# IGNF/MAESTRO

Hardware: AMD Instinct MI355X
Metric: MAE-pretrain tiles/sec (higher is better)
Workload: dtype bf16

## Files before the change

### include/maestro_hip.h

```cpp
#ifndef MAESTRO_HIP_H
#define MAESTRO_HIP_H
#include <stddef.h>
#include <stdint.h>
#ifdef __cplusplus
extern "C" {
#endif

const char* mh_last_error(void);
int mh_version(void);

#define MH_GEMM_OUT_F32 1
#define MH_GEMM_BIAS 2
#define MH_GEMM_GELU 4
#define MH_GEMM_RESIDUAL 8
#define MH_GEMM_DGELU 16
#define MH_GEMM_ATOMIC 32
#define MH_GEMM_COLSUM 64
#define MH_GEMM_AUX_DGELU 128
#define MH_GEMM_MULAUX 256
#define MH_GEMM_AUX_U8 1024
#define MH_GEMM_C8_E5M2 512
#define MH_GEMM_FP8_TILE_256 2048
#define MH_GEMM_FP8_TILE_128 4096
#define MH_GEMM_FP8_TILE_128D 8192
int mh_gemm_bf16(int layout, int M, int N, int K, const void* A, int lda, const void* B, int ldb, void* C, int ldc,
                 int flags, const float* bias, const float* res, int ldr, const void* aux_in, void* aux_out,
                 int ldaux, float* colsum, void* stream);

enum { MH_TILE_AUTO = -1, MH_TILE_REG_128 = 0, MH_TILE_DMA_256 = 1, MH_TILE_DMA_256x128 = 2, MH_TILE_DMA_128x256 = 3,
       MH_TILE_DMA_128 = 4, MH_TILE_DMA_128x4 = 5, MH_TILE_DMA_256_LOCKSTEP = 6, MH_TILE_PP_128 = 7,
       MH_TILE_PP_128_DIAG1 = 8, MH_TILE_PP_128_DIAG2 = 9, MH_TILE_PP_128_DIAG3 = 10,
       MH_TILE_PP_128_DIAG4 = 11, MH_TILE_PP_128_DIAG5 = 12,
       MH_TILE_REG_64 = 13, MH_TILE_REG_192 = 14,
       MH_TILE_SK_192 = 15, MH_TILE_SK_256 = 16,
       MH_TILE_SK_DMA_256 = 17  };
int mh_gemm_bf16_tile(int tile, int layout, int M, int N, int K, const void* A, int lda, const void* B, int ldb, void* C,
                      int ldc, int flags, const float* bias, const float* res, int ldr, const void* aux_in, void* aux_out,
                      int ldaux, float* colsum, void* stream);

#define MH_GEMM_FAMILY_DMA 1
#define MH_GEMM_FAMILY_PP 2
#define MH_GEMM_FAMILY_192 4
#define MH_GEMM_FAMILY_ALL 7
int mh_gemm_bf16_resolve_tile(int tile, int families, int layout, int M, int N, int K, int lda, int ldb, int ldc, int ldr,
                              int ldaux, int flags);

long mh_gemm_sk_workspace(int tile, int grid);
int mh_gemm_bf16_sk(int tile, int layout, int M, int N, int K, const void* A, int lda, const void* B, int ldb, void* C, int ldc,
                    int flags, const float* bias, const float* res, int ldr, void* workspace, long workspace_bytes, int grid,
                    void* stream);

typedef struct MhGroupedGemm {
    const void* A; const void* B; void* C;
    int M, N, K, lda, ldb, ldc, reserved, accumulate;
} MhGroupedGemm;
int mh_gemm_grouped_tn(const MhGroupedGemm* table_device, int n_problems, const uint32_t* tile_queues, int queue_len,
                       void* stream);

enum { MH_FP8_E4M3 = 0, MH_FP8_E5M2 = 1 };
int mh_gemm_fp8(int M, int N, int K, const void* A8, int lda, int a_format, const void* B8, int ldb, void* C, int ldc,
                int flags, const float* descale_a, const float* descale_b, const float* bias, const float* res, int ldr,
                const void* aux_in, void* aux_out, int ldaux, float* colsum, void* c8, int ldc8, const float* c8_scale,
                float* c8_amax, void* stream);
#define MH_FP8_AMAX_SUBSLOTS 32
#define MH_FP8_AMAX_STRIDE 64
#define MH_FP8_AMAX_PITCH (MH_FP8_AMAX_SUBSLOTS * MH_FP8_AMAX_STRIDE)
typedef struct MhQuantJob {
    const void* src; void* dst; void* dst_t;
    long n;
    int rows, cols, slot, is_f32, format, reserved;
} MhQuantJob;
int mh_quant_batched(const MhQuantJob* jobs_device, const unsigned long* items_device, int n_items, const float* scale,
                     float* amax, int mode, void* stream);
int mh_fp8_update_scales(float* amax, float* scale, float* descale, int n, float format_max, int margin_log2, void* stream);
int mh_gemm_mx(int M, int N, int K, const void* A8, int lda, const void* sa, int ldsa, const void* B8, int ldb, const void* sb,
               int ldsb, void* C, int ldc, int flags, const float* bias, const float* res, int ldr, const void* aux_in,
               void* aux_out, int ldaux, float* colsum, void* c8, int ldc8, void* c8_scales, int ldc8s, void* stream);
typedef struct MhQuantMxJob {
    const void* src; void* dst; void* scales;
    int rows, cols, ld_src, ld_dst, ld_s, reserved;
} MhQuantMxJob;
int mh_quant_mx_batched(const MhQuantMxJob* jobs_host, int n_jobs, const MhQuantMxJob* jobs_device, const unsigned long* items_device,
                        int n_items, void* stream);
typedef struct MhTransposeJob { const void* src; void* dst; int rows, cols; } MhTransposeJob;
int mh_transpose_u8_batched(const MhTransposeJob* jobs_device, const unsigned long* items_device, int n_items, void* stream);

int mh_layernorm_fwd(const float* x, int x_L, int x_off, const float* gamma, const float* beta, void* y, int y_L,
                     int y_off, int y_is_f32, float* mean, float* rstd, int B, int n, int dim, float eps, void* stream);
int mh_layernorm_fwd_fp8(const float* x, int x_L, int x_off, const float* gamma, const float* beta, void* y, int y_L,
                         int y_off, float* mean, float* rstd, int B, int n, int dim, float eps, void* y8,
                         const float* y8_scale, float* y8_amax, void* stream);
int mh_layernorm_fwd_mx(const float* x, int x_L, int x_off, const float* gamma, const float* beta, void* y, int y_L, int y_off,
                        float* mean, float* rstd, int B, int n, int dim, float eps, void* y8, void* y8_scales, int ld_y8s,
                        void* stream);
int mh_layernorm_bwd(const void* dy, int dy_L, int dy_off, int dy_is_f32, const float* x, int x_L, int x_off,
                     const float* gamma, const float* mean, const float* rstd, const float* dres, float* dx,
                     void* dx_bf16, float* dgamma, float* dbeta, float* dcol, float* workspace, int B, int n, int dim,
                     void* stream);
long mh_layernorm_bwd_workspace(int rows, int dim);
int mh_layernorm_bwd_partial(const void* dy, int dy_L, int dy_off, int dy_is_f32, const float* x, int x_L, int x_off,
                             const float* gamma, const float* mean, const float* rstd, const float* dres, float* dx,
                             void* dx_bf16, float* workspace, int B, int n, int dim, void* stream);
#define MH_COLSUM_ROWS 16
typedef struct {
    const float* src;
    float* dst;
    int rows, cols, ld, reserved;
} MhColsumJob;
int mh_colsum_batched(const MhColsumJob* jobs_device, int n_jobs, const uint64_t* blocks_device, int n_blocks, void* stream);
#define MH_ORDERED_ROWS 16
#define MH_ORDERED_ADD 1
typedef struct MhOrderedJob {
    const float* src;
    float* dst;
    int rows, cols, ld, flags;
} MhOrderedJob;
int mh_reduce_ordered(const MhOrderedJob* jobs_host, const MhOrderedJob* jobs_device, int n_jobs, const uint64_t* blocks_device,
                      int n_blocks, void* stream);

int mh_attn_fwd(const void* qkv, void* out, float* lse, int B, int N, int H, int D, float scale, void* stream);
int mh_attn_bwd(const void* qkv, const void* out, const void* dout, const float* lse, float* delta, void* dqkv,
                int B, int N, int H, int D, float scale, void* stream);
int mh_patchify(const float* img, void* cols, float* target, int BD, int Ctot, int S, int P, int Kpad,
                const int* norm_bands, int n_norm_groups, int normalise, int rescale_elev, void* stream);
int mh_patchify_bands(const float* img, void* cols, float* target, int BD, int Csrc, int c0, int Ctot, int S, int P, int Kpad,
                      const int* norm_bands, int n_norm_groups, int normalise, int rescale_elev, void* stream);

int mh_groupnorm_stats(const float* y, float* partial, float* stats, int BD, int L, int E, float eps, void* stream);
int mh_groupnorm_partial_size(int BD, int L, int E);
int mh_embed_finish(const float* y, const float* stats, const float* gamma, const float* beta, const float* pos,
                    const float* date, int date_rows, int date_off, float* xg, int B, int D, int L, int E, int tok_off,
                    int Lgroup, void* stream);
int mh_embed_finish_bwd(const float* dxg, const float* y, const float* stats, const float* gamma, void* dyc,
                        float* dgamma, float* dbeta, float* sums, int B, int D, int L, int E, int tok_off, int Lgroup,
                        void* stream);
int mh_embed_bwd_partial_rows(int BD, int L);
int mh_embed_finish_bwd_det(const float* dxg, const float* y, const float* stats, const float* gamma, void* dyc,
                            float* param_partial, float* blk_sums, float* sums, int B, int D, int L, int E, int tok_off, int Lgroup,
                            void* stream);
int mh_embed_bwd_cs_rows(long rows);
int mh_embed_finish_bwd_ends(const float* dx, const int* inv, int n_vis, const float* y, const float* stats, const float* gamma,
                             void* dyc, float* dgamma, float* dbeta, float* sums, float* cs_partial, int B, int D, int L, int E,
                             int tok_off, int Lgroup, void* stream);
int mh_date_features(const int16_t* dates, const int16_t* ref_date, float* out, int B, int D, int rows, int row_off,
                     float fac, void* stream);
int mh_resize(const float* in, float* out, long planes, int Hin, int Win, int Hout, int Wout, int mode, void* stream);
int mh_dihedral(const void* in, void* out, const uint8_t* flags, int B, long planes, int S, int elem_bytes, void* stream);
#define MH_RAW_U8 0
#define MH_RAW_I16 1
#define MH_RAW_U16 2
#define MH_RAW_F32 3
#define MH_SELECT_MAX_WINDOW 64
int mh_select_dates(const void* raw, int raw_code, const unsigned char* mask, int Cm, int mask_floor, const short* dates,
                    const int* t_start, const int* t_win, int w_max, const double* scores, float* out, short* out_dates,
                    int* out_index, int B, int Tmax, int nd, long n_elem, int n_pix, int log_scale, float norm_fac, void* stream);
int mh_rescale_elev(const float* img, float* out, int BD, int C, int S, void* stream);
int mh_depatchify(const float* patches, float* img, int BD, int C, int S, int P, void* stream);

int mh_mask_select(const float* noise, const uint8_t* struct_mask, int* visible_idx, int* masked_idx, int* inv,
                   uint8_t* mask, int B, int L, int k, void* stream);
int mh_gather_rows(const float* src, const int* idx, float* dst, int B, int src_L, int n_idx, int dim, int dst_L,
                   int dst_off, void* stream);
int mh_gather_rows_cs_rows(long rows);
int mh_gather_rows_bf16_cs(const float* src, const int* idx, void* dst16, float* cs_partial, int B, int src_L, int n_idx, int dim,
                           void* stream);
int mh_scatter_rows(const float* ddst, const int* idx, float* dsrc, int B, int src_L, int n_idx, int dim, int dst_L,
                    int dst_off, void* stream);
int mh_expand_rows(const float* src, const int* inv, float* dst, int B, int L, int n, int dim, void* stream);
int mh_unmask_assemble(const float* y, const int* inv, const float* mask_token, const int* tok_slot, const float* pos,
                       const float* date, const int* date_row, int n_date_rows, float* xdec, int B, int L, int n_vis,
                       int Dd, void* stream);
int mh_unmask_token_grad(const float* dxdec, const uint8_t* mask, const int* tok_slot, float* dmask_token, int B, int L,
                         int Dd, int slot, int t_lo, int t_hi, void* stream);
int mh_unmask_assemble_per_sample(const float* y, const int* inv, const float* mask_token, const int* tok_slot_bl,
                                  const float* pos, const float* date, const int* date_row, int n_date_rows, float* xdec,
                                  int B, int L, int n_vis, int Dd, void* stream);
int mh_unmask_token_grad_per_sample(const float* dxdec, const uint8_t* mask, const int* tok_slot_bl, float* dmask_token, int B,
                                    int L, int Dd, int slot, void* stream);
int mh_unmask_token_grad_partial_rows(long n_rows);
int mh_unmask_token_grad_det(const float* dxdec, const uint8_t* mask, const int* tok_slot, float* partial, int B, int L, int Dd,
                             int slot, int t_lo, int t_hi, void* stream);
int mh_unmask_token_grad_per_sample_det(const float* dxdec, const uint8_t* mask, const int* tok_slot_bl, float* partial, int B,
                                        int L, int Dd, int slot, void* stream);
int mh_count_masked(const uint8_t* mask, int B, int L, int t_lo, int t_hi, int* out, void* stream);
int mh_count_masked_elems(const uint8_t* mask, int B, int L, int t_lo, int t_hi, int* out, int mult, int accumulate, void* stream);

int mh_masked_loss(const float* rec, const float* target, const uint8_t* mask_group, const int* n_masked, float weight,
                   float* acc, void* drec, int B, int Lm, int Lgroup, int tok_off, int PPC, int p, void* stream);
int mh_masked_loss_bands(const float* rec, const float* target, const uint8_t* mask_group, const int* n_elems, float weight,
                         float* acc, void* drec, int B, int Lm, int Lgroup, int tok_off, int PPC, int p, int tgt_C, int tgt_c0,
                         int n_g, void* stream);
int mh_masked_loss_partial_size(int B, int Lm);
int mh_masked_loss_det(const float* rec, const float* target, const uint8_t* mask_group, const int* n_masked, float weight,
                       float* loss_partial, void* drec, int B, int Lm, int Lgroup, int tok_off, int PPC, int p, void* stream);
int mh_masked_loss_bands_det(const float* rec, const float* target, const uint8_t* mask_group, const int* n_elems, float weight,
                             float* loss_partial, void* drec, int B, int Lm, int Lgroup, int tok_off, int PPC, int p, int tgt_C,
                             int tgt_c0, int n_g, void* stream);
int mh_masked_loss_cs_rows(int B, int Lm);
int mh_masked_loss_cs(const float* rec, const float* target, const uint8_t* mask_group, const int* n_masked, float weight,
                      float* acc, void* drec, float* cs_partial, int B, int Lm, int Lgroup, int tok_off, int PPC, int p,
                      void* stream);
int mh_masked_loss_bands_cs(const float* rec, const float* target, const uint8_t* mask_group, const int* n_elems, float weight,
                            float* acc, void* drec, float* cs_partial, int B, int Lm, int Lgroup, int tok_off, int PPC, int p,
                            int tgt_C, int tgt_c0, int n_g, void* stream);

int mh_token_resize(const float* in, long in_rows, int in_off, float* out, long out_rows, int out_off, int B, int D, int h,
                    int H, int E, void* stream);
int mh_token_resize_bwd(const float* dout, long out_rows, int out_off, float* din, long in_rows, int in_off, int B, int D,
                        int h, int H, int E, int accumulate, void* stream);
int mh_attn_reduce_fwd(const void* kv, const float* query, float* out, float* lse, int n_batch, int T, int Lr, int dim,
                       int heads, void* stream);
int mh_attn_reduce_bwd(const void* kv, const float* query, const float* out, const float* lse, const float* dout, void* dkv,
                       float* dq_partial, int n_batch, int T, int Lr, int dim, int heads, void* stream);
long mh_attn_reduce_partial_rows(int n_seq);
int mh_mean_reduce_fwd(const float* x, float* out, int n_batch, int T, int Lr, int dim, void* stream);
int mh_mean_reduce_bwd(const float* dout, float* dx, int n_batch, int T, int Lr, int dim, void* stream);
int mh_head_linear_fwd(const float* x, const float* W, const float* bias, float* out, int B, int C, int E, void* stream);
int mh_head_linear_bwd(const float* x, const float* W, const float* dout, float* dx, float* dW, float* db, int B, int C, int E,
                       void* stream);
int mh_count_valid(const void* target, int target_bytes, long n, long missing_val, int* count, void* stream);
int mh_ce_loss(const float* logits, const void* target, int target_bytes, long missing_val, const int* n_valid, float* acc,
               void* dlogits, int dlogits_is_f32, int B, int g, int P, int C, int ld, void* stream);
int mh_bce_loss(const float* logits, const float* target, float missing_val, float* acc, float* dlogits, int B, int C,
                void* stream);
int mh_confusion_ce(const float* logits, const void* target, int target_bytes, long missing_val, long long* cm, int B, int g,
                    int P, int C, int ld, void* stream);
int mh_confusion_bce(const float* logits, const float* target, float missing_val, float logit_threshold, long long* cm, int B,
                     int C, void* stream);

int mh_colsum(const void* x, int x_is_f32, float* out, int M, int N, int ld, void* stream);
#define MH_COLSUM_PARTIAL_ROWS 256
int mh_colsum_partial_rows(int M);
int mh_colsum_partial(const void* x, int x_is_f32, float* partial, int M, int N, int ld, void* stream);
int mh_zero_spans(float* base, const long* spans_device, int n_spans, long max_len, void* stream);
int mh_scale_dev(float* x, long n, const float* scale, void* stream);
int mh_cast_bf16(const float* src, void* dst, long n, void* stream);
int mh_pack_rows_bf16(const float* w, void* dst, int E, int K, int Kpad, void* stream);
int mh_unpack_rows_add(const float* src, float* dst, int E, int K, int Kpad, void* stream);
int mh_adamw(float* p, const float* g, float* m, float* v, void* p_bf16, long n, float lr, float b1, float b2,
             float eps, float wd, int step, float grad_scale, void* stream);
int mh_adamw_fp8(float* p, const float* g, float* m, float* v, void* p_bf16, void* p_fp8, const short* slot_map,
                 const float* scale, float* amax, long n, float lr, float b1, float b2, float eps, float wd, int step,
                 float grad_scale, void* stream);
int mh_adamw_dev(float* p, const float* g, float* m, float* v, void* p_bf16, long n, float b1, float b2, float eps,
                 float wd, const float* hyper, void* stream);

#ifdef __cplusplus
}
#endif
#endif
```

### maestro_amd/csrc/gemm.hip

```cpp
#include "gemm_reg.hpp"

namespace {

template <bool A_KMAJOR, bool B_KMAJOR, int MT = 4>
__global__ __launch_bounds__(NT, MT == 2 ? 3 : 2) void gemm_kernel(GemmParams p) {
    static_assert(!A_KMAJOR || MT == 4, "the K-major A image is 128 columns wide");
    constexpr int TBM = 32 * MT, NA = MT;
    constexpr int A_BYTES = TBM * 128, B_BYTES = TILE_BYTES;
    __shared__ __attribute__((aligned(16))) unsigned char smem[2 * A_BYTES + 2 * B_BYTES];
    unsigned char* const sb = smem + 2 * A_BYTES;
    const int nwg = p.tiles_m * p.tiles_n;
    const int id = xcd_remap(blockIdx.x, nwg);
    constexpr int GROUP_M = MT == 2 ? 16 : 8;
    int tile_m, tile_n;
    raster_tile<GROUP_M>(p, id, tile_m, tile_n);
    const int m0 = tile_m * TBM, n0 = tile_n * BN;
    const int kbeg = blockIdx.y * p.k_per_split;
    const int kend = min(p.K, kbeg + p.k_per_split);
    const int nk = (kend - kbeg + BK - 1) / BK;

    const int w = threadIdx.x >> 6, l = threadIdx.x & 63;
    const int wm = (w >> 1) * (16 * MT), wn = (w & 1) * 64;

    f32x4 acc[4][MT];
#pragma unroll
    for (int j = 0; j < 4; ++j)
#pragma unroll
        for (int i = 0; i < MT; ++i) acc[j][i] = (f32x4){0.f, 0.f, 0.f, 0.f};

    u32x4 ra[NA], rb[4];
    auto mfma_block = [&](const bf16x8 (&fa)[MT], const bf16x8 (&fb)[4]) {
#pragma unroll
        for (int j = 0; j < 4; ++j)
#pragma unroll
            for (int i = 0; i < MT; ++i)
                acc[j][i] = __builtin_amdgcn_mfma_f32_16x16x32_bf16(fb[j], fa[i], acc[j][i], 0, 0, 0);
    };
    auto compute = [&](const unsigned char* ta, const unsigned char* tb) {
#pragma unroll
        for (int s = 0; s < 2; ++s) {
            bf16x8 fa[MT], fb[4];
#pragma unroll
            for (int i = 0; i < MT; ++i) fa[i] = read_frag<A_KMAJOR>(ta, wm + 16 * i, s);
#pragma unroll
            for (int j = 0; j < 4; ++j) fb[j] = read_frag<B_KMAJOR>(tb, wn + 16 * j, s);
            mfma_block(fa, fb);
        }
    };
    auto compute_half = [&](const unsigned char* ta, const unsigned char* tb, int s) {
        bf16x8 fa[MT], fb[4];
#pragma unroll
        for (int i = 0; i < MT; ++i) fa[i] = read_frag<A_KMAJOR>(ta, wm + 16 * i, s);
#pragma unroll
        for (int j = 0; j < 4; ++j) fb[j] = read_frag<B_KMAJOR>(tb, wn + 16 * j, s);
        __builtin_amdgcn_s_setprio(1);
        mfma_block(fa, fb);
        __builtin_amdgcn_s_setprio(0);
    };
    if (p.fast) {
        const __amdgpu_buffer_rsrc_t ra_src = __builtin_amdgcn_make_buffer_rsrc((void*)p.A, (short)0, (int)p.a_bytes, 0x00020000);
        const __amdgpu_buffer_rsrc_t rb_src = __builtin_amdgcn_make_buffer_rsrc((void*)p.B, (short)0, (int)p.b_bytes, 0x00020000);
        int va[NA], vb[4];
        tile_offsets<A_KMAJOR, NA>(p.lda, m0, va);
        tile_offsets<B_KMAJOR>(p.ldb, n0, vb);
        const int a_step = A_KMAJOR ? BK * p.lda * 2 : BK * 2;
        const int b_step = B_KMAJOR ? BK * p.ldb * 2 : BK * 2;
        int a_off = A_KMAJOR ? kbeg * p.lda * 2 : kbeg * 2;
        int b_off = B_KMAJOR ? kbeg * p.ldb * 2 : kbeg * 2;
        load_tile_fast(ra_src, va, a_off, ra);
        load_tile_fast(rb_src, vb, b_off, rb);
        store_tile<A_KMAJOR, NA>(smem, ra);
        store_tile<B_KMAJOR>(sb, rb);
        if (nk > 1) {
            a_off += a_step; b_off += b_step;
            load_tile_fast(ra_src, va, a_off, ra);
            load_tile_fast(rb_src, vb, b_off, rb);
        }
        __syncthreads();
        constexpr int NM = 4 * MT, NS = NA + 4;
        constexpr int NR = (A_KMAJOR ? 8 : MT) + (B_KMAJOR ? 8 : 4);
        int kt0 = 0;
        for (; kt0 + 2 < nk; ++kt0) {
            const int cur = kt0 & 1;
            const unsigned char* ta = smem + cur * A_BYTES;
            const unsigned char* tb = sb + cur * B_BYTES;
            bf16x8 fa[MT], fb[4];
#pragma unroll
            for (int i = 0; i < MT; ++i) fa[i] = read_frag<A_KMAJOR>(ta, wm + 16 * i, 0);
#pragma unroll
            for (int j = 0; j < 4; ++j) fb[j] = read_frag<B_KMAJOR>(tb, wn + 16 * j, 0);
            mfma_block(fa, fb);
            store_tile<A_KMAJOR, NA>(smem + (cur ^ 1) * A_BYTES, ra);
            store_tile<B_KMAJOR>(sb + (cur ^ 1) * B_BYTES, rb);
            a_off += a_step; b_off += b_step;
            load_tile_fast(ra_src, va, a_off, ra);
            load_tile_fast(rb_src, vb, b_off, rb);
#pragma unroll
            for (int i = 0; i < MT; ++i) fa[i] = read_frag<A_KMAJOR>(ta, wm + 16 * i, 1);
#pragma unroll
            for (int j = 0; j < 4; ++j) fb[j] = read_frag<B_KMAJOR>(tb, wn + 16 * j, 1);
            mfma_block(fa, fb);
            __builtin_amdgcn_sched_group_barrier(0x100, NR, 0);
#pragma unroll
            for (int r = 0; r < NS; ++r) {
                __builtin_amdgcn_sched_group_barrier(0x008, NM / NS, 0);
                __builtin_amdgcn_sched_group_barrier(0x200, 1, 0);
                __builtin_amdgcn_sched_group_barrier(0x020, 1, 0);
            }
            if constexpr (NM % NS != 0) __builtin_amdgcn_sched_group_barrier(0x008, NM - (NM / NS) * NS, 0);
            __builtin_amdgcn_sched_group_barrier(0x100, NR, 0);
            __builtin_amdgcn_sched_group_barrier(0x008, NM, 0);
            __syncthreads();
        }
        for (int kt = kt0; kt < nk; ++kt) {
            const int cur = kt & 1;
            const unsigned char* ta = smem + cur * A_BYTES;
            const unsigned char* tb = sb + cur * B_BYTES;
            compute_half(ta, tb, 0);
            if (kt + 1 < nk) {
                store_tile<A_KMAJOR, NA>(smem + (cur ^ 1) * A_BYTES, ra);
                store_tile<B_KMAJOR>(sb + (cur ^ 1) * B_BYTES, rb);
                if (kt + 2 < nk) {
                    a_off += a_step; b_off += b_step;
                    load_tile_fast(ra_src, va, a_off, ra);
                    load_tile_fast(rb_src, vb, b_off, rb);
                }
            }
            compute_half(ta, tb, 1);
            __syncthreads();
        }
    } else {
        unsigned char* ta = smem;
        unsigned char* tb = sb;
        load_tile<A_KMAJOR, NA>(p.A, p.lda, m0, p.M, kbeg, kend, ra);
        load_tile<B_KMAJOR>(p.B, p.ldb, n0, p.N, kbeg, kend, rb);
        store_tile<A_KMAJOR, NA>(ta, ra);
        store_tile<B_KMAJOR>(tb, rb);
        __syncthreads();
        for (int kt = 0; kt < nk; ++kt) {
            const bool more = kt + 1 < nk;
            if (more) {
                load_tile<A_KMAJOR, NA>(p.A, p.lda, m0, p.M, kbeg + (kt + 1) * BK, kend, ra);
                load_tile<B_KMAJOR>(p.B, p.ldb, n0, p.N, kbeg + (kt + 1) * BK, kend, rb);
            }
            compute(ta, tb);
            __syncthreads();
            if (more) {
                store_tile<A_KMAJOR, NA>(ta, ra);
                store_tile<B_KMAJOR>(tb, rb);
            }
            __syncthreads();
        }
    }

    float* st = reinterpret_cast<float*>(smem) + w * (32 * 68);
    if (p.flags & MH_GEMM_ATOMIC) gemm_epilogue_atomic<MT>(p, acc, st, m0 + wm, n0 + wn);
    else gemm_epilogue_store<MT>(p, acc, st, m0 + wm, n0 + wn);
}

}

static int gemm_reg_launch(int tile, int layout, GemmParams& p, hipStream_t s) {
    const int K = p.K;
    const int mt = tile == MH_TILE_REG_64 ? 2 : tile == MH_TILE_REG_192 ? 6 : 4;
    const int tbm = 32 * mt;
    p.tiles_m = ceil_div(p.M, tbm); p.tiles_n = ceil_div(p.N, BN);
    int splits = 1;
    if (p.flags & MH_GEMM_ATOMIC) {
        const int tiles = p.tiles_m * p.tiles_n;
        const int ksteps = ceil_div(K, BK);
        splits = max(1, min(min(512 / max(tiles, 1), ksteps / 4), 32));
    }
    const int ksteps_per = ceil_div(ceil_div(K, BK), splits);
    p.k_per_split = ksteps_per * BK;
    splits = ceil_div(K, p.k_per_split);
    const bool a_kmajor = layout == 2, b_kmajor = layout != 0;
    const long k_rows = (long)ceil_div(K, BK) * BK;
    const bool tail_ok = (a_kmajor && b_kmajor) || K % BK == 0;
    p.fast = tail_ok && gemm_in_reach((a_kmajor ? k_rows : (long)p.tiles_m * tbm) * p.lda * 2, 4096) &&
             gemm_in_reach((b_kmajor ? k_rows : (long)p.tiles_n * BN) * p.ldb * 2, 4096);
    gemm_set_extents(p, layout);
    dim3 grid(p.tiles_m * p.tiles_n, splits), block(NT);
    switch (layout * 8 + mt) {
        case 0 * 8 + 4: hipLaunchKernelGGL((gemm_kernel<false, false, 4>), grid, block, 0, s, p); break;
        case 0 * 8 + 2: hipLaunchKernelGGL((gemm_kernel<false, false, 2>), grid, block, 0, s, p); break;
        case 0 * 8 + 6: hipLaunchKernelGGL((gemm_kernel<false, false, 6>), grid, block, 0, s, p); break;
        case 1 * 8 + 4: hipLaunchKernelGGL((gemm_kernel<false, true, 4>), grid, block, 0, s, p); break;
        case 1 * 8 + 2: hipLaunchKernelGGL((gemm_kernel<false, true, 2>), grid, block, 0, s, p); break;
        case 1 * 8 + 6: hipLaunchKernelGGL((gemm_kernel<false, true, 6>), grid, block, 0, s, p); break;
        default: hipLaunchKernelGGL((gemm_kernel<true, true, 4>), grid, block, 0, s, p); break;
    }
    MH_LAUNCH_CHECK();
    return 0;
}

static int gemm_check_args(bool buffers, int tile, int layout, const GemmParams& p) {
    const int M = p.M, N = p.N, K = p.K, lda = p.lda, ldb = p.ldb, ldc = p.ldc, ldr = p.ldr, ldaux = p.ldaux, flags = p.flags;
    auto given = [&](const void* q) { return !buffers || q; };
    MH_CHECK_ARG(tile >= MH_TILE_AUTO && tile <= MH_TILE_REG_192, "mh_gemm_bf16: tile %d", tile);
    MH_CHECK_ARG(layout >= 0 && layout <= 2, "mh_gemm_bf16: layout %d", layout);
    MH_CHECK_ARG(!(flags & ~0x7ff), "mh_gemm_bf16: unknown flag bits 0x%x", flags & ~0x7ff);
    MH_CHECK_ARG(M > 0 && N > 0 && K > 0, "mh_gemm_bf16: empty problem %d %d %d", M, N, K);
    MH_CHECK_ARG(given(p.A) && given(p.B) && given(p.C), "mh_gemm_bf16: null operand");
    MH_CHECK_ARG(lda % 8 == 0 && ldb % 8 == 0, "mh_gemm_bf16: lda/ldb must be multiples of 8 (%d, %d)", lda, ldb);
    MH_CHECK_ARG(N % 4 == 0 && ldc % 4 == 0, "mh_gemm_bf16: N and ldc must be multiples of 4 (%d, %d)", N, ldc);
    MH_CHECK_ARG((flags & MH_GEMM_OUT_F32) || (N % 8 == 0 && ldc % 8 == 0), "mh_gemm_bf16: bf16 output needs N, ldc %% 8 == 0");
    MH_CHECK_ARG((flags & MH_GEMM_OUT_F32) || !(flags & MH_GEMM_RESIDUAL), "mh_gemm_bf16: residual epilogue needs f32 output");
    MH_CHECK_ARG(!(flags & MH_GEMM_OUT_F32) || !(flags & (MH_GEMM_GELU | MH_GEMM_DGELU | MH_GEMM_MULAUX)), "mh_gemm_bf16: GELU / aux epilogues need bf16 output");
    MH_CHECK_ARG(((uintptr_t)p.A | (uintptr_t)p.B | (uintptr_t)p.C) % 16 == 0, "mh_gemm_bf16: bases must be 16-B aligned");
    if (layout == 2) {
        MH_CHECK_ARG(M % 8 == 0 && N % 8 == 0, "mh_gemm_bf16: TN needs M, N multiples of 8 (%d, %d)", M, N);
    } else {
        MH_CHECK_ARG(K % 8 == 0, "mh_gemm_bf16: K must be a multiple of 8 (%d)", K);
        if (layout == 1) MH_CHECK_ARG(N % 8 == 0, "mh_gemm_bf16: NN needs N multiple of 8 (%d)", N);
    }
    MH_CHECK_ARG(!(flags & MH_GEMM_BIAS) || given(p.bias), "mh_gemm_bf16: bias flag without pointer");
    MH_CHECK_ARG(!(flags & MH_GEMM_RESIDUAL) || (given(p.res) && ldr % 4 == 0), "mh_gemm_bf16: residual needs pointer, ldr%%4==0");
    MH_CHECK_ARG(!(flags & (MH_GEMM_DGELU | MH_GEMM_MULAUX)) || (given(p.aux_in) && ldaux % 8 == 0), "mh_gemm_bf16: dgelu / mulaux need aux_in, ldaux %% 8 == 0");
    MH_CHECK_ARG(!(flags & MH_GEMM_AUX_DGELU) || ((flags & MH_GEMM_GELU) && given(p.aux_out)), "mh_gemm_bf16: aux_dgelu needs the GELU epilogue and aux_out");
    MH_CHECK_ARG(!((flags & MH_GEMM_DGELU) && (flags & MH_GEMM_MULAUX)), "mh_gemm_bf16: dgelu and mulaux exclude each other");
    MH_CHECK_ARG(!(flags & MH_GEMM_AUX_U8) || ((flags & (MH_GEMM_AUX_DGELU | MH_GEMM_MULAUX)) && !(flags & MH_GEMM_DGELU)),
                 "mh_gemm_bf16: MH_GEMM_AUX_U8 applies to the saved GELU derivative only (AUX_DGELU / MULAUX)");
    MH_CHECK_ARG(!(flags & MH_GEMM_GELU) || !p.aux_out || ldaux % 8 == 0, "mh_gemm_bf16: ldaux %% 8");
    MH_CHECK_ARG(!(flags & MH_GEMM_ATOMIC) || (flags & MH_GEMM_OUT_F32), "mh_gemm_bf16: atomic needs f32 output");
    MH_CHECK_ARG(!(flags & MH_GEMM_COLSUM) || (given(p.colsum) && !(flags & MH_GEMM_OUT_F32)), "mh_gemm_bf16: colsum needs a pointer and bf16 output");
    MH_CHECK_ARG(!(flags & MH_GEMM_ATOMIC) || !(flags & ~(MH_GEMM_ATOMIC | MH_GEMM_OUT_F32)),
                 "mh_gemm_bf16: atomic accumulate excludes other epilogues");
    return 0;
}

static bool prefer_dma(int layout, int M, int N, int K, int flags) {
    if (layout == 2 || (flags & MH_GEMM_ATOMIC) || K % 32 != 0 || K < 256) return false;
    const long tiles = (long)ceil_div(M, 256) * ceil_div(N, 256);
    if (tiles < 256) return false;
    const long waves = (tiles + 255) / 256;
    return 10 * tiles >= 9 * 256 * waves;
}

static int gemm_resolve(int tile, int families, int layout, const GemmParams& p) {
    const int M = p.M, N = p.N, K = p.K, flags = p.flags;
    if (tile >= MH_TILE_PP_128 && tile <= MH_TILE_PP_128_DIAG5) return gemm_pp_serves(tile, layout, p) ? tile : -2;
    if (tile > MH_TILE_REG_128 && tile < MH_TILE_PP_128) return gemm_dma_serves(tile, layout, p) ? tile : -2;
    if (tile != MH_TILE_AUTO)
        return layout != 2 && !(flags & MH_GEMM_COLSUM) ? tile : MH_TILE_REG_128;
    const bool dma = (families & MH_GEMM_FAMILY_DMA) && prefer_dma(layout, M, N, K, flags);
    const long t128 = (long)ceil_div(M, 128) * ceil_div(N, 128);
    if ((families & MH_GEMM_FAMILY_192) && !dma && layout != 2 && !(flags & (MH_GEMM_COLSUM | MH_GEMM_ATOMIC)) && K >= 1536 &&
        K % BK == 0 && t128 > 512 && t128 <= 576 && (long)ceil_div(M, 192) * ceil_div(N, 128) <= 512)
        return MH_TILE_REG_192;
    if ((families & MH_GEMM_FAMILY_PP) && !(flags & MH_GEMM_MULAUX) && layout == 0 && t128 >= 256 &&
        ((flags & MH_GEMM_GELU) ? t128 <= 2304 : (!dma || (K < 1024 && t128 <= 8192))) && gemm_pp_serves(MH_TILE_PP_128, layout, p))
        return MH_TILE_PP_128;
    if (dma && gemm_dma_serves(MH_TILE_DMA_256, layout, p)) return MH_TILE_DMA_256;
    return MH_TILE_REG_128;
}

extern "C" int mh_gemm_bf16_resolve_tile(int tile, int families, int layout, int M, int N, int K, int lda, int ldb, int ldc,
                                         int ldr, int ldaux, int flags) {
    GemmParams p;
    gemm_fill(p, M, N, K, nullptr, lda, nullptr, ldb, nullptr, ldc, flags, nullptr, nullptr, ldr, nullptr, nullptr, ldaux, nullptr);
    MH_CHECK_ARG(!(families & ~MH_GEMM_FAMILY_ALL), "mh_gemm_bf16_resolve_tile: unknown family bits 0x%x", families & ~MH_GEMM_FAMILY_ALL);
    if (const int rc = gemm_check_args(false, tile, layout, p)) return rc;
    return gemm_resolve(tile, families, layout, p);
}

extern "C" int mh_gemm_bf16_tile(int tile, int layout, int M, int N, int K, const void* A, int lda, const void* B, int ldb,
                                 void* C, int ldc, int flags, const float* bias, const float* res, int ldr,
                                 const void* aux_in, void* aux_out, int ldaux, float* colsum, void* stream) {
    GemmParams p;
    gemm_fill(p, M, N, K, A, lda, B, ldb, C, ldc, flags, bias, res, ldr, aux_in, aux_out, ldaux, colsum);
    if (const int rc = gemm_check_args(true, tile, layout, p)) return rc;
    const int run = gemm_resolve(tile, MH_GEMM_FAMILY_ALL, layout, p);
    if (run == -2) return -2;
    if (run >= MH_TILE_PP_128 && run <= MH_TILE_PP_128_DIAG5) return gemm_pp_launch(run, layout, p, (hipStream_t)stream);
    if (run > MH_TILE_REG_128 && run < MH_TILE_PP_128) return gemm_dma_launch(run, layout, p, (hipStream_t)stream);
    return gemm_reg_launch(run, layout, p, (hipStream_t)stream);
}

extern "C" int mh_gemm_bf16(int layout, int M, int N, int K, const void* A, int lda, const void* B, int ldb, void* C,
                            int ldc, int flags, const float* bias, const float* res, int ldr, const void* aux_in,
                            void* aux_out, int ldaux, float* colsum, void* stream) {
    return mh_gemm_bf16_tile(MH_TILE_AUTO, layout, M, N, K, A, lda, B, ldb, C, ldc, flags, bias, res, ldr, aux_in, aux_out,
                             ldaux, colsum, stream);
}
```

### maestro_amd/csrc/gemm_dma.hip

```cpp
#include "gemm_ring.hpp"

#ifndef MH_DMA_PRIO
#define MH_DMA_PRIO 0
#endif
#if MH_DMA_PRIO == 0
#define MH_PRIO_UP() __builtin_amdgcn_s_setprio(1)
#define MH_PRIO_DOWN() __builtin_amdgcn_s_setprio(0)
#else
#define MH_PRIO_UP() ((void)0)
#define MH_PRIO_DOWN() ((void)0)
#endif

namespace {

template <class T, bool A_KMAJOR, bool B_KMAJOR, int CALLER, bool STAGGER>
__device__ __forceinline__ void gemm_dma_tile(const GemmParams& p, int tile_m, int tile_n, int kbeg, int kend,
                                              unsigned char* smem) {
    constexpr int S = T::S, PA = T::PA, PB = T::PB, NW = T::NW;
    static_assert(T::LDS_BYTES >= NW * 32 * 68 * 4, "the ring doubles as epilogue staging");
    const int m0 = tile_m * T::BM, n0 = tile_n * T::BN;
    const int nk = (kend - kbeg + BK - 1) / BK;

    const int w = __builtin_amdgcn_readfirstlane(threadIdx.x >> 6), l = threadIdx.x & 63;
    constexpr int MT = T::MT;
    const int wm = (w / T::WN) * (16 * MT), wn = (w % T::WN) * 64;

    const __amdgpu_buffer_rsrc_t ra_src = __builtin_amdgcn_make_buffer_rsrc((void*)p.A, (short)0, (int)p.a_bytes, 0x00020000);
    const __amdgpu_buffer_rsrc_t rb_src = __builtin_amdgcn_make_buffer_rsrc((void*)p.B, (short)0, (int)p.b_bytes, 0x00020000);
    int va[PA], vb[PB];
    piece_offsets<A_KMAJOR, T::BM, NW, PA>(p.lda, m0, w, l, va);
    piece_offsets<B_KMAJOR, T::BN, NW, PB>(p.ldb, n0, w, l, vb);
    const int a_step = A_KMAJOR ? BK * p.lda * 2 : BK * 2;
    const int b_step = B_KMAJOR ? BK * p.ldb * 2 : BK * 2;
    const int a_off0 = A_KMAJOR ? kbeg * p.lda * 2 : kbeg * 2;
    const int b_off0 = B_KMAJOR ? kbeg * p.ldb * 2 : kbeg * 2;

    auto issue = [&](int t) {
        unsigned char* slot = smem + (t % S) * T::STAGE_BYTES;
#pragma unroll
        for (int h = 0; h < PA; ++h)
            __builtin_amdgcn_raw_ptr_buffer_load_lds(ra_src, (lds_void*)(slot + (w + NW * h) * 1024), 16, va[h],
                                                     a_off0 + t * a_step, 0, 0);
#pragma unroll
        for (int h = 0; h < PB; ++h)
            __builtin_amdgcn_raw_ptr_buffer_load_lds(rb_src, (lds_void*)(slot + T::A_BYTES + (w + NW * h) * 1024), 16, vb[h],
                                                     b_off0 + t * b_step, 0, 0);
    };

    f32x4 acc[4][MT];
#pragma unroll
    for (int j = 0; j < 4; ++j)
#pragma unroll
        for (int i = 0; i < MT; ++i) acc[j][i] = (f32x4){0.f, 0.f, 0.f, 0.f};

    for (int t = 0; t < S - 1 && t < nk; ++t) issue(t);

    auto wait_step = [&](int step) {
        const int younger = min(S - 2, nk - 1 - step);
        if (younger >= 2) wait_vmcnt<2 * (PA + PB)>();
        else if (younger == 1) wait_vmcnt<PA + PB>();
        else wait_vmcnt<0>();
    };
    bf16x8 fa[MT], fb[4];
    auto load_step = [&](int t) {
        const unsigned char* ta = smem + (t % S) * T::STAGE_BYTES;
        const unsigned char* tb = ta + T::A_BYTES;
#pragma unroll
        for (int j = 0; j < 4; ++j) fb[j] = read_frag<B_KMAJOR, T::BN>(tb, wn + 16 * j);
#pragma unroll
        for (int i = 0; i < MT; ++i) fa[i] = read_frag<A_KMAJOR, T::BM>(ta, wm + 16 * i);
        __builtin_amdgcn_sched_barrier(0);
        if (t + S - 1 < nk) issue(t + S - 1);
        __builtin_amdgcn_sched_barrier(0);
    };
    auto math_step = [&]() {
#pragma unroll
        for (int i = 0; i < MT; ++i)
#pragma unroll
            for (int j = 0; j < 4; ++j)
                acc[j][i] = __builtin_amdgcn_mfma_f32_16x16x32_bf16(fb[j], fa[i], acc[j][i], 0, 0, 0);
    };

    if constexpr (NW == 8 && STAGGER) {
        wait_step(0);
        __builtin_amdgcn_s_barrier();
#if MH_DMA_PRIO == 1
        if (w >= 4) __builtin_amdgcn_s_setprio(1);
#endif
        if (w < 4) {
            for (int t = 0; t < nk; ++t) {
                load_step(t);
                __builtin_amdgcn_s_barrier();
                __builtin_amdgcn_sched_barrier(0);
                MH_PRIO_UP(); math_step(); MH_PRIO_DOWN();
                if (t + 1 < nk) wait_step(t + 1);
                __builtin_amdgcn_s_barrier();
                __builtin_amdgcn_sched_barrier(0);
            }
        } else {
            __builtin_amdgcn_s_barrier();
            __builtin_amdgcn_sched_barrier(0);
            for (int t = 0; t < nk; ++t) {
                load_step(t);
                if (t + 1 < nk) wait_step(t + 1);
                __builtin_amdgcn_s_barrier();
                __builtin_amdgcn_sched_barrier(0);
                MH_PRIO_UP(); math_step(); MH_PRIO_DOWN();
                if (t + 1 < nk) {
                    __builtin_amdgcn_s_barrier();
                    __builtin_amdgcn_sched_barrier(0);
                }
            }
        }
    } else {
        for (int t = 0; t < nk; ++t) {
            wait_step(t);
            __builtin_amdgcn_s_barrier();
            load_step(t);
            math_step();
        }
        __builtin_amdgcn_s_barrier();
    }

    float* st = reinterpret_cast<float*>(smem) + w * (32 * 68);
    if (p.flags & MH_GEMM_ATOMIC) gemm_epilogue_atomic<MT>(p, acc, st, m0 + wm, n0 + wn);
    else gemm_epilogue_store<MT>(p, acc, st, m0 + wm, n0 + wn);
}

template <class T, bool A_KMAJOR, bool B_KMAJOR, bool STAGGER>
__global__ __launch_bounds__(T::NT, T::MIN_WG) void gemm_dma_kernel(GemmParams p) {
    __shared__ __attribute__((aligned(16))) unsigned char smem[T::LDS_BYTES];
    const int nwg = p.tiles_m * p.tiles_n;
    const int id = xcd_remap(blockIdx.x, nwg);
    int tile_m, tile_n;
    raster_tile<4>(p, id, tile_m, tile_n);
    const int kbeg = blockIdx.y * p.k_per_split;
    gemm_dma_tile<T, A_KMAJOR, B_KMAJOR, 0, STAGGER>(p, tile_m, tile_n, kbeg, min(p.K, kbeg + p.k_per_split), smem);
}

typedef Tile<2, 4, 4> T256;
typedef Tile<2, 2, 3> T256x128;
typedef Tile<1, 4, 3> T128x256;
typedef Tile<1, 2, 4> T128;
typedef Tile<2, 2, 4, 4> T128q;

template <class T, bool STAGGER>
__global__ __launch_bounds__(T::NT) void gemm_dma_grouped_tn_kernel(const MhGroupedGemm* __restrict__ table, int n_problems,
                                                                    const uint32_t* __restrict__ queues, int queue_len) {
    __shared__ __attribute__((aligned(16))) unsigned char smem[T::LDS_BYTES];
    const uint32_t e = queues[(size_t)(blockIdx.x & 7) * queue_len + (blockIdx.x >> 3)];
    if (e == 0xFFFFFFFFu || (int)(e >> 16) >= n_problems) return;
    const MhGroupedGemm g = table[e >> 16];
    GemmParams p;
    p.A = (const bf16_t*)g.A; p.B = (const bf16_t*)g.B; p.C = g.C;
    p.bias = nullptr; p.res = nullptr; p.aux_in = nullptr; p.aux_out = nullptr; p.colsum = nullptr;
    p.M = g.M; p.N = g.N; p.K = g.K; p.lda = g.lda; p.ldb = g.ldb; p.ldc = g.ldc; p.ldr = 0; p.ldaux = 0;
    p.flags = MH_GEMM_OUT_F32 | (g.accumulate ? MH_GEMM_ATOMIC : 0);
    p.tiles_m = (g.M + T::BM - 1) / T::BM; p.tiles_n = (g.N + T::BN - 1) / T::BN; p.k_per_split = g.K; p.fast = 1;
    p.a_bytes = (unsigned)(((long)(g.K - 1) * g.lda + g.M) * 2);
    p.b_bytes = (unsigned)(((long)(g.K - 1) * g.ldb + g.N) * 2);
    const int tile_m = (e >> 8) & 0xff, tile_n = e & 0xff;
    if (tile_m >= p.tiles_m || tile_n >= p.tiles_n) return;
    gemm_dma_tile<T, true, true, 1, STAGGER>(p, tile_m, tile_n, 0, g.K, smem);
}

template <class T>
void launch_dma(int layout, GemmParams& p, hipStream_t s, bool stagger = true) {
    const int K = p.K;
    p.tiles_m = ceil_div(p.M, T::BM); p.tiles_n = ceil_div(p.N, T::BN);
    int splits = 1;
    if (p.flags & MH_GEMM_ATOMIC) {
        const int tiles = p.tiles_m * p.tiles_n, ksteps = ceil_div(K, BK);
        const int slots = 256 * (T::LDS_BYTES > 80 * 1024 ? 1 : 2);
        splits = max(1, min(min(slots / max(tiles, 1), ksteps / 8), 32));
    }
    const int ksteps_per = ceil_div(ceil_div(K, BK), splits);
    p.k_per_split = ksteps_per * BK;
    splits = ceil_div(K, p.k_per_split);
    dim3 grid(p.tiles_m * p.tiles_n, splits), block(T::NT);
    if (T::NW == 8 && stagger) {
        switch (layout) {
            case 0: hipLaunchKernelGGL((gemm_dma_kernel<T, false, false, T::NW == 8>), grid, block, 0, s, p); break;
            case 1: hipLaunchKernelGGL((gemm_dma_kernel<T, false, true, T::NW == 8>), grid, block, 0, s, p); break;
            default: hipLaunchKernelGGL((gemm_dma_kernel<T, true, true, T::NW == 8>), grid, block, 0, s, p); break;
        }
        return;
    }
    switch (layout) {
        case 0: hipLaunchKernelGGL((gemm_dma_kernel<T, false, false, false>), grid, block, 0, s, p); break;
        case 1: hipLaunchKernelGGL((gemm_dma_kernel<T, false, true, false>), grid, block, 0, s, p); break;
        default: hipLaunchKernelGGL((gemm_dma_kernel<T, true, true, false>), grid, block, 0, s, p); break;
    }
}

}

extern "C" int mh_gemm_grouped_tn(const MhGroupedGemm* table_device, int n_problems, const uint32_t* tile_queues,
                                  int queue_len, void* stream) {
    MH_CHECK_ARG(table_device && tile_queues && n_problems > 0 && n_problems < 65536 && queue_len > 0,
                 "mh_gemm_grouped_tn: bad arguments");
    hipLaunchKernelGGL((gemm_dma_grouped_tn_kernel<T256, true>), dim3(8 * queue_len), dim3(T256::NT), 0, (hipStream_t)stream,
                       table_device, n_problems, tile_queues, queue_len);
    MH_LAUNCH_CHECK();
    return 0;
}

bool gemm_dma_serves(int tile, int layout, const GemmParams& p) {
    int bm, bn;
    switch (tile) {
        case MH_TILE_DMA_256: case MH_TILE_DMA_256_LOCKSTEP: bm = T256::BM; bn = T256::BN; break;
        case MH_TILE_DMA_256x128: bm = T256x128::BM; bn = T256x128::BN; break;
        case MH_TILE_DMA_128x256: bm = T128x256::BM; bn = T128x256::BN; break;
        case MH_TILE_DMA_128: case MH_TILE_DMA_128x4: bm = T128::BM; bn = T128::BN; break;
        default: return false;
    }
    const bool a_kmajor = layout == 2, b_kmajor = layout != 0;
    if ((!a_kmajor || !b_kmajor) && p.K % BK != 0) return false;
    const long k_rows = (long)ceil_div(p.K, BK) * BK;
    return gemm_in_reach((a_kmajor ? k_rows : (long)ceil_div(p.M, bm) * bm) * p.lda * 2) &&
           gemm_in_reach((b_kmajor ? k_rows : (long)ceil_div(p.N, bn) * bn) * p.ldb * 2);
}

int gemm_dma_launch(int tile, int layout, GemmParams& p, hipStream_t s) {
    p.fast = 1;
    gemm_set_extents(p, layout);
    switch (tile) {
        case MH_TILE_DMA_256: launch_dma<T256>(layout, p, s); break;
        case MH_TILE_DMA_256x128: launch_dma<T256x128>(layout, p, s); break;
        case MH_TILE_DMA_128x256: launch_dma<T128x256>(layout, p, s); break;
        case MH_TILE_DMA_128: launch_dma<T128>(layout, p, s); break;
        case MH_TILE_DMA_128x4: launch_dma<T128q>(layout, p, s); break;
        default: launch_dma<T256>(layout, p, s, false); break;
    }
    MH_LAUNCH_CHECK();
    return 0;
}
```

### maestro_amd/csrc/gemm_pp.hip

```cpp
#include "gemm_reg.hpp"
#include <type_traits>

#ifndef MH_PP_PRIO
#define MH_PP_PRIO 1
#endif

namespace {

enum { EPI_BF16 = 0, EPI_GELU = 1, EPI_MULAUX = 2, EPI_F32 = 3 };
constexpr int EPI_STEPS = 8;

__device__ __forceinline__ void swap16(uint32_t& a, uint32_t& b) {
    const u32x2 r = __builtin_amdgcn_permlane16_swap(a, b, false, false);
    a = r[0]; b = r[1];
}

template <bool B_KMAJOR, int EPI, int DIAG = 0>
__global__ __launch_bounds__(NT, 2) void gemm_pp_kernel(GemmParams p) {
    __shared__ __attribute__((aligned(16))) unsigned char smem[4 * TILE_BYTES];
    const int T = p.tiles_m * p.tiles_n, G = gridDim.x;
    const int x = blockIdx.x & 7, slot = blockIdx.x >> 3, per_x = G >> 3;
    const int q = T >> 3, r8 = T & 7;
    const int run0 = x < r8 ? x * (q + 1) : r8 * (q + 1) + (x - r8) * q;
    const int cnt = q + (x < r8 ? 1 : 0);
    if (slot >= cnt) return;
    const int n_my = (cnt - slot + per_x - 1) / per_x;
    const int nk = p.K / BK;
    auto coords = [&](int t, int& m0, int& n0) {
        int tm, tn;
        raster_tile<8>(p, run0 + slot + t * per_x, tm, tn);
        m0 = tm * BM;
        n0 = tn * BN;
    };

    const int tid = threadIdx.x, w = tid >> 6, l = tid & 63, g = l >> 4, lm = l & 15;
    const int wm = (w >> 1) * 64, wn = (w & 1) * 64;

    const __amdgpu_buffer_rsrc_t ra_src = __builtin_amdgcn_make_buffer_rsrc((void*)p.A, (short)0, (int)p.a_bytes, 0x00020000);
    const __amdgpu_buffer_rsrc_t rb_src = __builtin_amdgcn_make_buffer_rsrc((void*)p.B, (short)0, (int)p.b_bytes, 0x00020000);
    const int a_v0 = ((tid >> 3) * p.lda + (tid & 7) * 8) * 2;
    const int b_v0 = B_KMAJOR ? ((tid >> 4) * p.ldb + (tid & 15) * 8) * 2 : ((tid >> 3) * p.ldb + (tid & 7) * 8) * 2;
    const int a_i = 32 * p.lda * 2, b_i = (B_KMAJOR ? 16 : 32) * p.ldb * 2;
    const int a_step = BK * 2, b_step = B_KMAJOR ? BK * p.ldb * 2 : BK * 2;
    int ld_kt = 0, ld_m0, ld_n0, nx_m0, nx_n0;
    coords(0, ld_m0, ld_n0);
    coords(min(1, n_my - 1), nx_m0, nx_n0);
    u32x4 ra[4], rb[4];
    auto issue_loads = [&]() {
        const int a_t = ld_m0 * p.lda * 2, b_t = B_KMAJOR ? ld_n0 * 2 : ld_n0 * p.ldb * 2;
        const int a_k = ld_kt * a_step, b_k = ld_kt * b_step;
#pragma unroll
        for (int i = 0; i < 4; ++i) ra[i] = __builtin_amdgcn_raw_buffer_load_b128(ra_src, a_v0 + (a_t + i * a_i), a_k, 0);
#pragma unroll
        for (int i = 0; i < 4; ++i) rb[i] = __builtin_amdgcn_raw_buffer_load_b128(rb_src, b_v0 + (b_t + i * b_i), b_k, 0);
    };
    auto advance = [&]() {
        const bool wrap = ++ld_kt == nk;
        ld_kt = wrap ? 0 : ld_kt;
        ld_m0 = wrap ? nx_m0 : ld_m0;
        ld_n0 = wrap ? nx_n0 : ld_n0;
    };

    f32x4 acc[4][4], prev[4][4];
    int sidx = 0;

    const __amdgpu_buffer_rsrc_t rc_dst = __builtin_amdgcn_make_buffer_rsrc(
        p.C, (short)0, (int)(((long)(p.M - 1) * p.ldc + p.N) * (EPI == EPI_F32 ? 4 : 2)), 0x00020000);
    const __amdgpu_buffer_rsrc_t raux = __builtin_amdgcn_make_buffer_rsrc(
        EPI == EPI_GELU ? (void*)p.aux_out : EPI == EPI_MULAUX ? (void*)p.aux_in : (void*)p.res, (short)0,
        (int)(EPI == EPI_F32 ? ((long)(p.M - 1) * p.ldr + p.N) * 4 : EPI == EPI_BF16 ? 0 : (long)(p.M - 1) * p.ldaux + p.N), 0x00020000);
    const __amdgpu_buffer_rsrc_t rbias = __builtin_amdgcn_make_buffer_rsrc((void*)p.bias, (short)0, p.bias ? p.N * 4 : 0, 0x00020000);
    const __amdgpu_buffer_rsrc_t rcs = __builtin_amdgcn_make_buffer_rsrc(
        (void*)p.colsum, (short)0, EPI == EPI_MULAUX ? (int)((long)((p.M + 63) / 64) * p.N * 4) : 0, 0x00020000);
    const int w_s = __builtin_amdgcn_readfirstlane(w);
    int e_c = 0, e_aux = 0, e_bias = 0, e_cs = 0;
    f32x4 bias_x = {0, 0, 0, 0}, bias_y = {0, 0, 0, 0};
    f32x4 cs_x = {0, 0, 0, 0}, cs_y = {0, 0, 0, 0};
    u32x4 ld_x = {0, 0, 0, 0}, ld_y = {0, 0, 0, 0};
    auto epi_setup = [&](int m0, int n0) {
        int lane = __builtin_amdgcn_mbcnt_hi(~0u, __builtin_amdgcn_mbcnt_lo(~0u, 0u));
        asm volatile("" : "+v"(lane));
        const int g = lane >> 4, lm = lane & 15;
        const int wm = (w_s >> 1) * 64, wn = (w_s & 1) * 64;
        const int col_nat = wn + 4 * g;
        const int col_swp = wn + 4 * g + 12 * (g & 1);
        const int row = m0 + wm + lm;
        if constexpr (EPI == EPI_F32) {
            e_c = (row * p.ldc + n0 + col_nat) * 4;
            e_aux = (row * p.ldr + n0 + col_nat) * 4;
        } else {
            e_c = (row * p.ldc + n0 + col_swp) * 2;
            e_aux = row * p.ldaux + n0 + (EPI == EPI_GELU ? col_swp : col_nat);
        }
        e_bias = (n0 + col_nat) * 4;
        e_cs = (((m0 + wm) >> 6) * p.N + n0 + col_nat) * 4;
    };
    auto epi_loads = [&](auto cc) {
        constexpr int c = decltype(cc)::value, jp = c >> 2, i = c & 3;
        if constexpr (DIAG == 1) return;
        if constexpr (EPI == EPI_GELU || EPI == EPI_F32) {
            if constexpr (i == 0) {
                bias_x = __builtin_bit_cast(f32x4, __builtin_amdgcn_raw_buffer_load_b128(rbias, e_bias + 128 * jp, 0, 0));
                bias_y = __builtin_bit_cast(f32x4, __builtin_amdgcn_raw_buffer_load_b128(rbias, e_bias + 128 * jp + 64, 0, 0));
            }
        }
        if constexpr (EPI == EPI_F32) {
            const int o = e_aux + (16 * i * p.ldr + 32 * jp) * 4;
            ld_x = __builtin_amdgcn_raw_buffer_load_b128(raux, o, 0, 0);
            ld_y = __builtin_amdgcn_raw_buffer_load_b128(raux, o + 64, 0, 0);
        }
        if constexpr (EPI == EPI_MULAUX) {
            const int o = e_aux + 16 * i * p.ldaux + 32 * jp;
            ld_x[0] = __builtin_amdgcn_raw_buffer_load_b32(raux, o, 0, 0);
            ld_y[0] = __builtin_amdgcn_raw_buffer_load_b32(raux, o + 16, 0, 0);
        }
    };
    auto epi_math = [&](auto cc, const f32x4 (&src)[4][4]) {
        constexpr int c = decltype(cc)::value, jp = c >> 2, i = c & 3;
        f32x4 vx = src[2 * jp][i], vy = src[2 * jp + 1][i];
        if constexpr (DIAG == 1) {
            asm volatile("" ::"v"(vx), "v"(vy));
            return;
        }
        if constexpr (EPI == EPI_F32) {
            const int o = e_c + (16 * i * p.ldc + 32 * jp) * 4;
            vx = vx + (bias_x + __builtin_bit_cast(f32x4, ld_x));
            vy = vy + (bias_y + __builtin_bit_cast(f32x4, ld_y));
            __builtin_amdgcn_raw_buffer_store_b128(__builtin_bit_cast(u32x4, vx), rc_dst, o, 0, 0);
            __builtin_amdgcn_raw_buffer_store_b128(__builtin_bit_cast(u32x4, vy), rc_dst, o + 64, 0, 0);
            return;
        } else {
            if constexpr (EPI == EPI_GELU) {
                vx += bias_x; vy += bias_y;
                f32x4 cx, dx, cy, dy;
                if constexpr (DIAG == 3) { cx = vx; dx = vx; cy = vy; dy = vy; }
                else { gelu_cdf_pdf4(vx, cx, dx); gelu_cdf_pdf4(vy, cy, dy); }
                const f32x4 gx = vx * dx + cx, gy = vy * dy + cy;
                uint32_t bx = 0, by = 0;
#pragma unroll
                for (int e = 0; e < 4; ++e) {
                    bx = __builtin_amdgcn_cvt_pk_u8_f32(__builtin_fmaf(gx[e], 200.f, 26.f), e, bx);
                    by = __builtin_amdgcn_cvt_pk_u8_f32(__builtin_fmaf(gy[e], 200.f, 26.f), e, by);
                }
                swap16(bx, by);
                if constexpr (DIAG == 2) asm volatile("" ::"v"(bx), "v"(by));
                else __builtin_amdgcn_raw_buffer_store_b64((u32x2){bx, by}, raux, e_aux + 16 * i * p.ldaux + 32 * jp, 0, 0);
                vx *= cx; vy *= cy;
            }
            if constexpr (EPI == EPI_MULAUX) {
                vx *= unpack_dgelu_u8x4(ld_x[0]);
                vy *= unpack_dgelu_u8x4(ld_y[0]);
                if constexpr (i == 0) { cs_x = vx; cs_y = vy; } else { cs_x += vx; cs_y += vy; }
                if constexpr (i == 3) {
#pragma unroll
                    for (int o = 1; o < 16; o <<= 1) {
#pragma unroll
                        for (int e = 0; e < 4; ++e) {
                            cs_x[e] += __shfl_xor(cs_x[e], o, 64);
                            cs_y[e] += __shfl_xor(cs_y[e], o, 64);
                        }
                    }
                    __builtin_amdgcn_raw_buffer_store_b128(__builtin_bit_cast(u32x4, cs_x), rcs, e_cs + 128 * jp, 0, 0);
                    __builtin_amdgcn_raw_buffer_store_b128(__builtin_bit_cast(u32x4, cs_y), rcs, e_cs + 128 * jp + 64, 0, 0);
                }
            }
            uint32_t x0 = pack_bf2(vx[0], vx[1]), x1 = pack_bf2(vx[2], vx[3]);
            uint32_t y0 = pack_bf2(vy[0], vy[1]), y1 = pack_bf2(vy[2], vy[3]);
            swap16(x0, y0);
            swap16(x1, y1);
            if constexpr (DIAG == 2) asm volatile("" ::"v"(x0), "v"(x1), "v"(y0), "v"(y1));
            else __builtin_amdgcn_raw_buffer_store_b128((u32x4){x0, x1, y0, y1}, rc_dst, e_c + (16 * i * p.ldc + 32 * jp) * 2, 0, 0);
        }
    };

    auto kstep = [&](auto first_c, auto chunk_c) {
        constexpr bool FIRST = decltype(first_c)::value;
        constexpr int CHUNK = decltype(chunk_c)::value;
        const int cur = sidx & 1;
        const unsigned char* ta = smem + cur * TILE_BYTES;
        const unsigned char* tb = smem + (2 + cur) * TILE_BYTES;
        bf16x8 fa[4], fb[4];
#if MH_PP_PRIO == 2
        __builtin_amdgcn_s_setprio(1);
#endif
#pragma unroll
        for (int i = 0; i < 4; ++i) fa[i] = read_frag<false>(ta, wm + 16 * i, 0);
#pragma unroll
        for (int j = 0; j < 4; ++j) fb[j] = read_frag<B_KMAJOR>(tb, wn + 16 * j, 0);
        if constexpr (CHUNK >= 0) epi_loads(chunk_c);
#if MH_PP_PRIO == 1 || MH_PP_PRIO == 3
        __builtin_amdgcn_s_setprio(MH_PP_PRIO);
#endif
#pragma unroll
        for (int j = 0; j < 4; ++j)
#pragma unroll
            for (int i = 0; i < 4; ++i)
                acc[j][i] = __builtin_amdgcn_mfma_f32_16x16x32_bf16(fb[j], fa[i], FIRST ? (f32x4){0.f, 0.f, 0.f, 0.f} : acc[j][i], 0, 0, 0);
        store_tile<false>(smem + (cur ^ 1) * TILE_BYTES, ra);
        store_tile<B_KMAJOR>(smem + (2 + (cur ^ 1)) * TILE_BYTES, rb);
        issue_loads();
#pragma unroll
        for (int i = 0; i < 4; ++i) fa[i] = read_frag<false>(ta, wm + 16 * i, 1);
#pragma unroll
        for (int j = 0; j < 4; ++j) fb[j] = read_frag<B_KMAJOR>(tb, wn + 16 * j, 1);
#pragma unroll
        for (int j = 0; j < 4; ++j)
#pragma unroll
            for (int i = 0; i < 4; ++i)
                acc[j][i] = __builtin_amdgcn_mfma_f32_16x16x32_bf16(fb[j], fa[i], acc[j][i], 0, 0, 0);
        if constexpr (CHUNK >= 0) epi_math(chunk_c, prev);
        constexpr int NV0 = CHUNK < 0 ? 0 : EPI == EPI_GELU ? 14 : EPI == EPI_MULAUX ? 6 : EPI == EPI_F32 ? 2 : 2;
        constexpr int NV = DIAG == 4 ? NV0 : DIAG == 5 ? (NV0 * 4 + 6) / 7 : 0;
        constexpr int NR = DIAG == 5 ? NV0 * 2 : 0;
        __builtin_amdgcn_sched_group_barrier(0x100, B_KMAJOR ? 12 : 8, 0);
        if constexpr (NR > 0) __builtin_amdgcn_sched_group_barrier(0x402, NR, 0);
        constexpr int NL = CHUNK < 0 ? 0 : (EPI == EPI_F32 || EPI == EPI_MULAUX ? 2 : 0) + ((EPI == EPI_F32 || EPI == EPI_GELU) && (CHUNK & 3) == 0 ? 2 : 0);
        if constexpr (NL > 0) __builtin_amdgcn_sched_group_barrier(0x020, NL, 0);
#pragma unroll
        for (int r = 0; r < 8; ++r) {
            __builtin_amdgcn_sched_group_barrier(0x008, 2, 0);
            __builtin_amdgcn_sched_group_barrier(0x200, 1, 0);
            __builtin_amdgcn_sched_group_barrier(0x020, 1, 0);
            if constexpr (NV > 0) __builtin_amdgcn_sched_group_barrier(0x402, NV, 0);
        }
        __builtin_amdgcn_sched_group_barrier(0x100, B_KMAJOR ? 12 : 8, 0);
        if constexpr (NR > 0) __builtin_amdgcn_sched_group_barrier(0x402, NR, 0);
#pragma unroll
        for (int r = 0; r < 8; ++r) {
            __builtin_amdgcn_sched_group_barrier(0x008, 2, 0);
            if constexpr (NV > 0) __builtin_amdgcn_sched_group_barrier(0x402, NV, 0);
        }
        ++sidx;
#if MH_PP_PRIO
        __builtin_amdgcn_s_setprio(0);
#endif
        __syncthreads();
        advance();
    };
    using std::integral_constant;
    constexpr integral_constant<bool, true> kFirst{};
    constexpr integral_constant<bool, false> kNext{};
    constexpr integral_constant<int, -1> kNone{};

    issue_loads(); advance();
    store_tile<false>(smem, ra);
    store_tile<B_KMAJOR>(smem + 2 * TILE_BYTES, rb);
    issue_loads();
    __syncthreads();
    advance();

    int cm0, cn0;
    coords(0, cm0, cn0);
    kstep(kFirst, kNone);
    for (int kt = 1; kt < nk; ++kt) kstep(kNext, kNone);
    for (int t = 1; t < n_my; ++t) {
#pragma unroll
        for (int j = 0; j < 4; ++j)
#pragma unroll
            for (int i = 0; i < 4; ++i) prev[j][i] = acc[j][i];
        epi_setup(cm0, cn0);
        coords(t, cm0, cn0);
        coords(min(t + 1, n_my - 1), nx_m0, nx_n0);
        kstep(kFirst, integral_constant<int, 0>{});
        kstep(kNext, integral_constant<int, 1>{});
        kstep(kNext, integral_constant<int, 2>{});
        kstep(kNext, integral_constant<int, 3>{});
        kstep(kNext, integral_constant<int, 4>{});
        kstep(kNext, integral_constant<int, 5>{});
        kstep(kNext, integral_constant<int, 6>{});
        kstep(kNext, integral_constant<int, 7>{});
        for (int kt = EPI_STEPS; kt < nk; ++kt) kstep(kNext, kNone);
    }
    epi_setup(cm0, cn0);
    if constexpr (DIAG == 0 && (EPI == EPI_F32 || EPI == EPI_MULAUX)) {
        u32x4 tx[8], ty[8];
        f32x4 tbx[2] = {{0, 0, 0, 0}, {0, 0, 0, 0}}, tby[2] = {{0, 0, 0, 0}, {0, 0, 0, 0}};
        auto fetch = [&](auto cc) {
            constexpr int c = decltype(cc)::value;
            epi_loads(cc);
            tx[c] = ld_x; ty[c] = ld_y;
            if constexpr ((c & 3) == 0) { tbx[c >> 2] = bias_x; tby[c >> 2] = bias_y; }
        };
        auto finish = [&](auto cc) {
            constexpr int c = decltype(cc)::value;
            ld_x = tx[c]; ld_y = ty[c]; bias_x = tbx[c >> 2]; bias_y = tby[c >> 2];
            epi_math(cc, acc);
        };
        fetch(integral_constant<int, 0>{}); fetch(integral_constant<int, 1>{}); fetch(integral_constant<int, 2>{});
        fetch(integral_constant<int, 3>{}); fetch(integral_constant<int, 4>{}); fetch(integral_constant<int, 5>{});
        fetch(integral_constant<int, 6>{}); fetch(integral_constant<int, 7>{});
        finish(integral_constant<int, 0>{}); finish(integral_constant<int, 1>{}); finish(integral_constant<int, 2>{});
        finish(integral_constant<int, 3>{}); finish(integral_constant<int, 4>{}); finish(integral_constant<int, 5>{});
        finish(integral_constant<int, 6>{}); finish(integral_constant<int, 7>{});
    } else {
        auto tail = [&](auto cc) { epi_loads(cc); epi_math(cc, acc); };
        tail(integral_constant<int, 0>{}); tail(integral_constant<int, 1>{}); tail(integral_constant<int, 2>{});
        tail(integral_constant<int, 3>{}); tail(integral_constant<int, 4>{}); tail(integral_constant<int, 5>{});
        tail(integral_constant<int, 6>{}); tail(integral_constant<int, 7>{});
    }
}

template <bool B_KMAJOR>
void launch_pp(int epi, int grid, const GemmParams& p, hipStream_t s, int diag = 0) {
    dim3 g(grid), b(NT);
#ifdef MH_DIAG_TILES
    if constexpr (!B_KMAJOR) {
        if (diag == 1 && epi == EPI_GELU) { hipLaunchKernelGGL((gemm_pp_kernel<false, EPI_GELU, 1>), g, b, 0, s, p); return; }
        if (diag == 2 && epi == EPI_GELU) { hipLaunchKernelGGL((gemm_pp_kernel<false, EPI_GELU, 2>), g, b, 0, s, p); return; }
        if (diag == 3 && epi == EPI_GELU) { hipLaunchKernelGGL((gemm_pp_kernel<false, EPI_GELU, 3>), g, b, 0, s, p); return; }
        if (diag == 4 && epi == EPI_GELU) { hipLaunchKernelGGL((gemm_pp_kernel<false, EPI_GELU, 4>), g, b, 0, s, p); return; }
        if (diag == 5 && epi == EPI_GELU) { hipLaunchKernelGGL((gemm_pp_kernel<false, EPI_GELU, 5>), g, b, 0, s, p); return; }
        if (diag == 1 && epi == EPI_BF16) { hipLaunchKernelGGL((gemm_pp_kernel<false, EPI_BF16, 1>), g, b, 0, s, p); return; }
    }
#else
    (void)diag;
#endif
    switch (epi) {
        case EPI_BF16: hipLaunchKernelGGL((gemm_pp_kernel<B_KMAJOR, EPI_BF16>), g, b, 0, s, p); break;
        case EPI_GELU: hipLaunchKernelGGL((gemm_pp_kernel<B_KMAJOR, EPI_GELU>), g, b, 0, s, p); break;
        case EPI_MULAUX: hipLaunchKernelGGL((gemm_pp_kernel<B_KMAJOR, EPI_MULAUX>), g, b, 0, s, p); break;
        default: hipLaunchKernelGGL((gemm_pp_kernel<B_KMAJOR, EPI_F32>), g, b, 0, s, p); break;
    }
}

}

static int pp_epilogue(int flags) {
    if (flags == 0) return EPI_BF16;
    if (flags == (MH_GEMM_BIAS | MH_GEMM_GELU | MH_GEMM_AUX_DGELU | MH_GEMM_AUX_U8)) return EPI_GELU;
    if (flags == (MH_GEMM_MULAUX | MH_GEMM_AUX_U8 | MH_GEMM_COLSUM)) return EPI_MULAUX;
    if (flags == (MH_GEMM_OUT_F32 | MH_GEMM_BIAS | MH_GEMM_RESIDUAL)) return EPI_F32;
    return -1;
}

bool gemm_pp_serves(int tile, int layout, const GemmParams& p) {
    const int epi = pp_epilogue(p.flags), diag = tile - MH_TILE_PP_128;
#ifndef MH_DIAG_TILES
    if (diag != 0) return false;
#else
    if (diag != 0 && (layout != 0 || !(epi == EPI_GELU || (epi == EPI_BF16 && diag == 1)))) return false;
#endif
    if (epi < 0 || layout == 2 || p.K % BK != 0 || p.K < EPI_STEPS * BK || p.N % BN != 0) return false;
    const long rows = (long)ceil_div(p.M, BM) * BM;
    return gemm_in_reach(rows * p.lda * 2) && gemm_in_reach((long)(layout == 1 ? p.K : p.N) * p.ldb * 2) &&
           gemm_in_reach(rows * p.ldc * (epi == EPI_F32 ? 4 : 2)) && gemm_in_reach(epi == EPI_F32 ? rows * p.ldr * 4 : rows * p.ldaux);
}

int gemm_pp_launch(int tile, int layout, GemmParams& p, hipStream_t stream) {
    p.tiles_m = ceil_div(p.M, BM); p.tiles_n = p.N / BN; p.k_per_split = p.K; p.fast = 1;
    gemm_set_extents(p, layout);
    const int tiles = p.tiles_m * p.tiles_n;
#ifndef MH_PP_TILES_PER_WG
#define MH_PP_TILES_PER_WG 0
#endif
    int grid = tiles >= 512 ? 512 : (tiles + 7) / 8 * 8;
    if (MH_PP_TILES_PER_WG > 0) grid = max(grid, ((tiles + MH_PP_TILES_PER_WG - 1) / MH_PP_TILES_PER_WG + 7) / 8 * 8);
    if (layout == 1) launch_pp<true>(pp_epilogue(p.flags), grid, p, stream);
    else launch_pp<false>(pp_epilogue(p.flags), grid, p, stream, tile - MH_TILE_PP_128);
    MH_LAUNCH_CHECK();
    return 0;
}
```

### maestro_amd/engine.py

```python

from __future__ import annotations

import contextlib
import gc
import os
import weakref
import time

import torch
from torch import nn

from maestro_amd import hip
from maestro_amd.fp8 import mx_scale_cols, resolve_scaling
from maestro_amd.layers.utils import draw_struct_masks

F32, BF16, I32, U8 = torch.float32, torch.bfloat16, torch.int32, torch.uint8
_NEVER = object()
_ROCTX = os.environ.get("MAESTRO_ROCTX", "0") == "1"
RING = 4
ALIGN = 64


class ParamStore:

# ... 154 lines not shown
            s, x_in, x_mid, x_out = self.saved[l], self.xs[2 * l], self.xs[2 * l + 1], self.xs[2 * l + 2]
            if self.f8 is not None:
                self._forward_layer_fp8(l, attn, ff, s, x_in, x_mid, x_out)
                continue
            proj = attn.to_out[0]
            hip.layernorm_fwd(x_in, M, 0, attn.norm.weight, attn.norm.bias, s["h1"], M, 0, s["mean1"], s["rstd1"], 1, M, dim)
            hip.gemm(hip.GEMM_NT, M, 3 * inner, dim, s["h1"], dim, ps.h(attn.to_qkv.weight), dim, s["qkv"], 3 * inner)
            hip.attn_fwd(s["qkv"], s["o"], s["lse"], self.Bn, self.N, self.H, self.Dh, attn.scale)
            hip.gemm(hip.GEMM_NT, M, dim, inner, s["o"], inner, ps.h(proj.weight), inner, x_mid, dim,
                     hip.OUT_F32 | hip.BIAS | hip.RESIDUAL, bias=proj.bias, res=x_in, ldr=dim)
            ln2, fc1, fc2 = ff.net[0], ff.net[1], ff.net[4]
            hip.layernorm_fwd(x_mid, M, 0, ln2.weight, ln2.bias, s["h2"], M, 0, s["mean2"], s["rstd2"], 1, M, dim)
            hip.gemm(hip.GEMM_NT, M, mlp, dim, s["h2"], dim, ps.h(fc1.weight), dim, s["act"], mlp,
                     hip.BIAS | hip.GELU | hip.AUX_DGELU | eng.aux_flag, bias=fc1.bias, aux_out=s["hpre"], ldaux=mlp)
            hip.gemm(hip.GEMM_NT, M, dim, mlp, s["act"], mlp, ps.h(fc2.weight), mlp, x_out, dim,
                     hip.OUT_F32 | hip.BIAS | hip.RESIDUAL, bias=fc2.bias, res=x_mid, ldr=dim)

    def _forward_layer_fp8(self, l, attn, ff, s, x_in, x_mid, x_out) -> None:
        eng, M, dim, mlp, inner = self.eng, self.M, self.dim, self.mlp, self.inner
        plan, f = eng.fp8, self.f8[l]
        proj, ln2, fc1, fc2 = attn.to_out[0], ff.net[0], ff.net[1], ff.net[4]
        fc1_flags = hip.BIAS | hip.GELU | hip.AUX_DGELU | eng.aux_flag
        res_flags = hip.OUT_F32 | hip.BIAS | hip.RESIDUAL
        if plan.scaling == "mx":
            ws = plan.w_scales
            ld = lambda t: t.stride(0)
            hip.layernorm_fwd_mx(x_in, M, 0, attn.norm.weight, attn.norm.bias, s["h1"], M, 0, s["mean1"], s["rstd1"], 1, M, dim,
                                 f["h1"], f["mx_h1"], ld(f["mx_h1"]))
            hip.gemm_mx(M, 3 * inner, dim, f["h1"], dim, f["mx_h1"], ld(f["mx_h1"]), f["w_qkv"], dim, ws(f["sw_qkv"]), dim // 32,
                        s["qkv"], 3 * inner)
            hip.attn_fwd(s["qkv"], s["o"], s["lse"], self.Bn, self.N, self.H, self.Dh, attn.scale)
            plan.quantize_mx(s["o"], f["o"], f["mx_o"])
            hip.gemm_mx(M, dim, inner, f["o"], inner, f["mx_o"], ld(f["mx_o"]), f["w_proj"], inner, ws(f["sw_proj"]), inner // 32,
                        x_mid, dim, flags=res_flags, bias=proj.bias, res=x_in, ldr=dim)
            hip.layernorm_fwd_mx(x_mid, M, 0, ln2.weight, ln2.bias, s["h2"], M, 0, s["mean2"], s["rstd2"], 1, M, dim, f["h2"],
                                 f["mx_h2"], ld(f["mx_h2"]))
            hip.gemm_mx(M, mlp, dim, f["h2"], dim, f["mx_h2"], ld(f["mx_h2"]), f["w_fc1"], dim, ws(f["sw_fc1"]), dim // 32,
                        s["act"], mlp, flags=fc1_flags, bias=fc1.bias, aux_out=s["hpre"], ldaux=mlp, c8=f["act"], ldc8=mlp,
                        c8_scales=f["mx_act"], ldc8s=ld(f["mx_act"]))
            hip.gemm_mx(M, dim, mlp, f["act"], mlp, f["mx_act"], ld(f["mx_act"]), f["w_fc2"], mlp, ws(f["sw_fc2"]), mlp // 32,
                        x_out, dim, flags=res_flags, bias=fc2.bias, res=x_mid, ldr=dim)
            return
        hip.layernorm_fwd_fp8(x_in, M, 0, attn.norm.weight, attn.norm.bias, s["h1"], M, 0, s["mean1"], s["rstd1"], 1, M, dim,
                              f["h1"], plan.a_scale(f["s_h1"]), plan.a_amax(f["s_h1"]))
        hip.gemm_fp8(M, 3 * inner, dim, f["h1"], dim, f["w_qkv"], dim, s["qkv"], 3 * inner, plan.a_descale(f["s_h1"]),
                     plan.w_descale(f["sw_qkv"]))
        hip.attn_fwd(s["qkv"], s["o"], s["lse"], self.Bn, self.N, self.H, self.Dh, attn.scale)
        plan.quantize(s["o"], f["o"], f["s_o"])
        hip.gemm_fp8(M, dim, inner, f["o"], inner, f["w_proj"], inner, x_mid, dim, plan.a_descale(f["s_o"]),
                     plan.w_descale(f["sw_proj"]), flags=res_flags, bias=proj.bias, res=x_in, ldr=dim)
        hip.layernorm_fwd_fp8(x_mid, M, 0, ln2.weight, ln2.bias, s["h2"], M, 0, s["mean2"], s["rstd2"], 1, M, dim, f["h2"],
                              plan.a_scale(f["s_h2"]), plan.a_amax(f["s_h2"]))
        hip.gemm_fp8(M, mlp, dim, f["h2"], dim, f["w_fc1"], dim, s["act"], mlp, plan.a_descale(f["s_h2"]),
                     plan.w_descale(f["sw_fc1"]), flags=fc1_flags, bias=fc1.bias, aux_out=s["hpre"],
                     ldaux=mlp, c8=f["act"], ldc8=mlp, c8_scale=plan.a_scale(f["s_act"]), c8_amax=plan.a_amax(f["s_act"]))
        hip.gemm_fp8(M, dim, mlp, f["act"], mlp, f["w_fc2"], mlp, x_out, dim, plan.a_descale(f["s_act"]),
                     plan.w_descale(f["sw_fc2"]), flags=res_flags, bias=fc2.bias, res=x_mid, ldr=dim)

    def reduce_jobs(self, lo: int = 0, hi: int | None = None) -> list:
        ps, dim, mlp, jobs = self.eng.store, self.dim, self.mlp, []
        for l in range(lo, self.depth if hi is None else hi):
            attn, ff = self.t.layers[l]
            s, ln2, fc1, proj = self.saved[l], ff.net[0], ff.net[1], attn.to_out[0]
            jobs.append((s["cs"], ps.g(fc1.bias), self.cs_rows, mlp, mlp))
            for ws, norm, bias in ((s["ws2"], ln2, ps.g(proj.bias)),
                                   (s["ws1"], attn.norm, ps.g(self.t.layers[l - 1][1].net[4].bias) if l > 0 else None)):
                flat = ws.view(-1)
                jobs.append((flat, ps.g(norm.weight), self.ln_rows, dim, 3 * dim))
                jobs.append((flat[dim:], ps.g(norm.bias), self.ln_rows, dim, 3 * dim))
                if bias is not None:
                    jobs.append((flat[2 * dim:], bias, self.ln_rows, dim, 3 * dim))
        return jobs

    def wgrad_problems(self, lo: int = 0, hi: int | None = None) -> list:
        ps, M = self.eng.store, self.M
        dim, mlp, inner = self.dim, self.mlp, self.inner
        out = []
        for l in range(lo, self.depth if hi is None else hi):
            attn, ff = self.t.layers[l]
            s, fc1, fc2, proj = self.saved[l], ff.net[1], ff.net[4], attn.to_out[0]
            out += [(s["gy16"], s["act"], ps.g(fc2.weight), dim, mlp, M, dim, mlp, mlp),
                    (s["dh"], s["h2"], ps.g(fc1.weight), mlp, dim, M, mlp, dim, dim),
                    (s["gmid16"], s["o"], ps.g(proj.weight), dim, inner, M, dim, inner, inner),
                    (s["dqkv"], s["h1"], ps.g(attn.to_qkv.weight), 3 * inner, dim, M, 3 * inner, dim, dim)]
        return out

    def backward(self, dx_out: torch.Tensor, hi: int | None = None, lo: int = 0, defer: bool = False, ready: bool = True):
        eng, ps, M = self.eng, self.eng.store, self.M
        dim, mlp, inner = self.dim, self.mlp, self.inner
        AT = hip.OUT_F32 | hip.ATOMIC
        cur = dx_out
        hi = self.depth if hi is None else hi
        cur16 = self.saved[hi - 1]["gy16"] if hi > 0 else self.dx0_16
        for l in reversed(range(lo, hi)):
            attn, ff = self.t.layers[l]
            s, x_in, x_mid = self.saved[l], self.xs[2 * l], self.xs[2 * l + 1]
            ln2, fc1, fc2 = ff.net[0], ff.net[1], ff.net[4]
            proj = attn.to_out[0]
            cur16, mid16, dh, dqkv = s["gy16"], s["gmid16"], s["dh"], s["dqkv"]
            mid = self.dxa if cur is not self.dxa else self.dxb
            nxt = self.dxa if mid is not self.dxa else self.dxb
            nxt16 = self.saved[l - 1]["gy16"] if l > 0 else self.dx0_16
            f = self.f8[l] if self.f8 is not None and self.f8[l]["dgrad"] else None
            plan = getattr(eng, "fp8", None)
            f8 = f is not None and plan.grad_ready
            if f is not None:
                plan.quantize_grad(cur16, f["gy8"], f["g_gy"])
            if f8:
                hip.gemm_fp8(M, mlp, dim, f["gy8"], dim, f["wt_fc2"], dim, dh, mlp, plan.g_descale(f["g_gy"]),
                             plan.w_descale(f["sw_fc2"]), flags=hip.MULAUX | hip.COLSUM | hip.C8_E5M2 | eng.aux_flag, a_format=hip.FP8_E5M2,
                             aux_in=s["hpre"], ldaux=mlp, colsum=s["cs"] if defer else self.cs_ws, c8=f["dh8"], ldc8=mlp,
                             c8_scale=plan.g_scale(f["g_dh"]), c8_amax=plan.g_amax(f["g_dh"]))
            else:
                hip.gemm(hip.GEMM_NN, M, mlp, dim, cur16, dim, ps.h(fc2.weight), mlp, dh, mlp, hip.MULAUX | hip.COLSUM | eng.aux_flag,
                         aux_in=s["hpre"], ldaux=mlp, colsum=s["cs"] if defer else self.cs_ws)
                if f is not None:
                    plan.quantize_grad(dh, f["dh8"], f["g_dh"])
            if not defer:
                hip.colsum(self.cs_ws, ps.g(fc1.bias), self.cs_rows, mlp, mlp)
                hip.gemm(hip.GEMM_TN, dim, mlp, M, cur16, dim, s["act"], mlp, ps.g(fc2.weight), mlp, AT)
                hip.gemm(hip.GEMM_TN, mlp, dim, M, dh, mlp, s["h2"], dim, ps.g(fc1.weight), dim, AT)
            if f8:
                hip.gemm_fp8(M, dim, mlp, f["dh8"], mlp, f["wt_fc1"], mlp, self.dh2, dim, plan.g_descale(f["g_dh"]),
                             plan.w_descale(f["sw_fc1"]), a_format=hip.FP8_E5M2)
            else:
                hip.gemm(hip.GEMM_NN, M, dim, mlp, dh, mlp, ps.h(fc1.weight), dim, self.dh2, dim)
            if defer:
                hip.layernorm_bwd_partial(self.dh2, M, 0, x_mid, M, 0, ln2.weight, s["mean2"], s["rstd2"], cur, mid, mid16, s["ws2"],
                                          1, M, dim)
            else:
                hip.layernorm_bwd(self.dh2, M, 0, x_mid, M, 0, ln2.weight, s["mean2"], s["rstd2"], cur, mid, mid16,
                                  ps.g(ln2.weight), ps.g(ln2.bias), ps.g(proj.bias), self.ln_ws, 1, M, dim)
            if f is not None:
                plan.quantize_grad(mid16, f["mid8"], f["g_mid"])
            if f8:
                hip.gemm_fp8(M, inner, dim, f["mid8"], dim, f["wt_proj"], dim, self.do, inner, plan.g_descale(f["g_mid"]),
                             plan.w_descale(f["sw_proj"]), a_format=hip.FP8_E5M2)
            else:
                hip.gemm(hip.GEMM_NN, M, inner, dim, mid16, dim, ps.h(proj.weight), inner, self.do, inner)
            if not defer:
                hip.gemm(hip.GEMM_TN, dim, inner, M, mid16, dim, s["o"], inner, ps.g(proj.weight), inner, AT)
            hip.attn_bwd(s["qkv"], s["o"], self.do, s["lse"], self.delta, dqkv, self.Bn, self.N, self.H, self.Dh, attn.scale)
            if not defer:
                hip.gemm(hip.GEMM_TN, 3 * inner, dim, M, dqkv, 3 * inner, s["h1"], dim, ps.g(attn.to_qkv.weight), dim, AT)
            if f is not None:
                plan.quantize_grad(dqkv, f["dqkv8"], f["g_dqkv"])
            if f8:
                hip.gemm_fp8(M, dim, 3 * inner, f["dqkv8"], 3 * inner, f["wt_qkv"], 3 * inner, self.dh2, dim,
                             plan.g_descale(f["g_dqkv"]), plan.w_descale(f["sw_qkv"]), a_format=hip.FP8_E5M2)
            else:
                hip.gemm(hip.GEMM_NN, M, dim, 3 * inner, dqkv, 3 * inner, ps.h(attn.to_qkv.weight), dim, self.dh2, dim)
            prev_fc2_bias = ps.g(self.t.layers[l - 1][1].net[4].bias) if l > 0 else None
            if defer:
                hip.layernorm_bwd_partial(self.dh2, M, 0, x_in, M, 0, attn.norm.weight, s["mean1"], s["rstd1"], mid, nxt, nxt16,
                                          s["ws1"], 1, M, dim)
            else:
                hip.layernorm_bwd(self.dh2, M, 0, x_in, M, 0, attn.norm.weight, s["mean1"], s["rstd1"], mid, nxt, nxt16,
                                  ps.g(attn.norm.weight), ps.g(attn.norm.bias), prev_fc2_bias, self.ln_ws, 1, M, dim)
            cur, cur16 = nxt, nxt16
            if ready:
                eng._grads_ready(self.t.layers[l])
        return cur, cur16


class PatchEmbedEnd:

    def __init__(self, eng: "EngineBase", s) -> None:
        self.eng, self.s = eng, s
        m, dev, E = eng.model, eng.device, eng.E
        e = lambda *sh, dt=F32: torch.empty(*sh, dtype=dt, device=dev)
        z = lambda *sh, dt=F32: torch.zeros(*sh, dtype=dt, device=dev)
        T, BD = s.Beff * s.n_tok, s.Beff * s.D
        self.buf = dict(
            cols=e(T, s.Kpad, dt=BF16), yconv=e(T, E), gn_partial=e(hip.groupnorm_partial_size(BD, s.L, E)), gn_stats=e(BD, 2),
            gn_sums=e(BD, 2), pos_enc=m.pos_enc_rows[s.name].to(dev), norm_bands=torch.tensor(s.norm_bands, dtype=I32, device=dev),
            w_conv16=z(E, s.Kpad, dt=BF16), dw_conv=z(E, s.Kpad), dyc=e(T, E, dt=BF16),
            pe=m.patch_embed[s.embed].patchify_bands[s.gi])

    def pack(self) -> None:
        b, s = self.buf, self.s
        hip.pack_rows_bf16(b["pe"].conv.weight, b["w_conv16"], self.eng.E, s.K, s.Kpad)

    def forward(self, batch: dict, gbuf: dict, xg: torch.Tensor, Lgroup: int, target=None, normalise: bool = False) -> None:
        eng, s, b = self.eng, self.s, self.buf
        m, B, E = eng.model, eng.B, eng.E
        BD, T = s.Beff * s.D, s.Beff * s.n_tok
        if s.G == 1 and target is not None:
            hip.patchify(batch[s.src], b["cols"], target, BD, s.C, s.S, s.P, s.Kpad, b["norm_bands"], len(s.norm_bands),
                         normalise, s.rescale_elev)
        else:
            hip.patchify_bands(batch[s.src], b["cols"], None, BD, s.C_src, s.c0, s.C, s.S, s.P, s.Kpad, None, 0, False,
                               s.rescale_elev)
            if target is not None and s.gi == 0:
                k_src = s.C_src * s.P * s.P
                hip.patchify_bands(batch[s.src], None, target, BD, s.C_src, 0, s.C_src, s.S, s.P, (k_src + 7) // 8 * 8,
                                   b["norm_bands"], len(s.norm_bands), normalise, s.rescale_elev)
        dates, ref_date = batch[f"{s.src}_dates"], batch["ref_date"]
        if s.D != s.Dates:
            hip.date_features(dates, ref_date, gbuf["dates"].view(B, s.Dates, 8), B, s.Dates, s.Dates, 0, m.fac_date_enc)
        else:
            hip.date_features(dates, ref_date, gbuf["dates"], B, s.D, gbuf["n_dates"], s.date_off, m.fac_date_enc)
        pe = b["pe"]
        hip.gemm(hip.GEMM_NT, T, E, s.Kpad, b["cols"], s.Kpad, b["w_conv16"], s.Kpad, b["yconv"], E, hip.OUT_F32 | hip.BIAS,
                 bias=pe.conv.bias)
        hip.groupnorm_stats(b["yconv"], b["gn_partial"], b["gn_stats"], BD, s.L, E)
        hip.embed_finish(b["yconv"], b["gn_stats"], pe.norm.weight, pe.norm.bias, b["pos_enc"], gbuf["dates"], gbuf["n_dates"],
                         s.date_off, xg, s.Beff, s.D, s.L, E, s.tok_off, Lgroup)

    def backward(self, dxg: torch.Tensor, Lgroup: int, clear_dw: bool, defer_wgrad: bool = False) -> None:
        eng, s, b = self.eng, self.s, self.buf
        ps, E, pe, T = eng.store, eng.E, b["pe"], s.Beff * s.n_tok
        if getattr(eng, "deterministic", False):
            return self._backward_det(dxg, Lgroup)
        hip.embed_finish_bwd(dxg, b["yconv"], b["gn_stats"], pe.norm.weight, b["dyc"], ps.g(pe.norm.weight), ps.g(pe.norm.bias),
                             b["gn_sums"], s.Beff, s.D, s.L, E, s.tok_off, Lgroup)
        if not defer_wgrad:
            self._wgrad_in_line(clear_dw)
        hip.colsum(b["dyc"], ps.g(pe.conv.bias), T, E, E)

    def _wgrad_in_line(self, clear_dw: bool) -> None:
        eng, s, b = self.eng, self.s, self.buf
        E, T = eng.E, s.Beff * s.n_tok
        if clear_dw:
            b["dw_conv"].zero_()
        hip.gemm(hip.GEMM_TN, E, s.Kpad, T, b["dyc"], E, b["cols"], s.Kpad, b["dw_conv"], s.Kpad, hip.OUT_F32 | hip.ATOMIC)
        hip.unpack_rows_add(b["dw_conv"], eng.store.g(b["pe"].conv.weight), E, s.K, s.Kpad)

    def wgrad_problem(self) -> tuple:
        b, s, E = self.buf, self.s, self.eng.E
        return (b["dyc"], b["cols"], b["dw_conv"], E, s.Kpad, s.Beff * s.n_tok, E, s.Kpad, s.Kpad)

    def cs_buffer(self) -> torch.Tensor:
        b, s = self.buf, self.s
        if b.get("dyc_cs") is None:
            b["dyc_cs"] = torch.empty(hip.embed_bwd_cs_rows(s.Beff * s.n_tok), self.eng.E, dtype=F32, device=self.eng.device)
        return b["dyc_cs"]

    def backward_ends(self, dx: torch.Tensor, inv, n_vis: int, Lgroup: int, defer_wgrad: bool, clear_dw: bool) -> None:
        eng, s, b = self.eng, self.s, self.buf
        ps, E, pe = eng.store, eng.E, b["pe"]
        hip.embed_finish_bwd_ends(dx, inv, n_vis, b["yconv"], b["gn_stats"], pe.norm.weight, b["dyc"], ps.g(pe.norm.weight),
                                  ps.g(pe.norm.bias), b["gn_sums"], self.cs_buffer(), s.Beff, s.D, s.L, E, s.tok_off, Lgroup)
        if not defer_wgrad:
            self._wgrad_in_line(clear_dw)

    def _backward_det(self, dxg: torch.Tensor, Lgroup: int) -> None:
        eng, s, b = self.eng, self.s, self.buf
        ps, E, pe, T = eng.store, eng.E, b["pe"], s.Beff * s.n_tok

        def make():
            e = lambda *sh: torch.empty(*sh, dtype=F32, device=eng.device)
            rows, S, cr = hip.embed_bwd_partial_rows(s.Beff * s.D, s.L), hip.det_slices(T), hip.colsum_partial_rows(T)
            w = dict(gn=e(rows, 2 * E), blk=e(rows, 2), slabs=e(S, E, s.Kpad), cs=e(cr, E))
            flat = w["gn"].view(-1)
            return w, [(flat, ps.g(pe.norm.weight), rows, E, 2 * E), (flat[E:], ps.g(pe.norm.bias), rows, E, 2 * E),
                       (w["slabs"].view(-1), b["dw_conv"].view(-1), S, E * s.Kpad, E * s.Kpad),
                       (w["cs"].view(-1), ps.g(pe.conv.bias), cr, E, E)]
        w = eng._det_site("bwd", ("embed", s.name), make)
        hip.embed_finish_bwd_det(dxg, b["yconv"], b["gn_stats"], pe.norm.weight, b["dyc"], w["gn"], w["blk"], b["gn_sums"], s.Beff,
                                 s.D, s.L, E, s.tok_off, Lgroup)
        hip.gemm_tn_slabs(E, s.Kpad, T, b["dyc"], E, b["cols"], s.Kpad, w["slabs"])
        hip.colsum_partial(b["dyc"], w["cs"], T, E, E)


_RETIRED_GRAPHS: list = []


def resolve_deterministic(flag: bool | None = None) -> bool:
    if flag is None:
        return os.environ.get("MAESTRO_DETERMINISTIC", "0") == "1"
    return bool(flag)


def training_warm_passes() -> int:
    return 0 if _PROCESS_WARMED else max(0, int(os.environ.get("MAESTRO_WARM_PASSES", "6")))


def _retire_graphs(graphs: dict) -> None:
    if graphs:
        _RETIRED_GRAPHS.append(dict(graphs))
        graphs.clear()


def drain_retired_graphs() -> None:
    if _RETIRED_GRAPHS:
        torch.cuda.synchronize()
        _RETIRED_GRAPHS.clear()


_PROCESS_WARMED = False


class EngineBase:

    def _init_runtime(self, device, n_side_streams: int) -> None:
        self.device = device
        self.grad_hook = None
        self.use_graphs = os.environ.get("MAESTRO_GRAPHS", "1") != "0"
        self.tie_order = os.environ.get("MAESTRO_TIE_ORDER", "stable")
        self.multi_stream = True
        self.group_streams = os.environ.get("MAESTRO_GROUP_STREAMS") != "0"
        self.tune_gemm = os.environ.get("MAESTRO_TUNE", "0") == "1"
        self.instep_tune = (os.environ.get("MAESTRO_INSTEP_TUNE", "0") == "1" and not self.tune_gemm
                            and not any(os.environ.get(k) for k in ("MH_GEMM_TILE", "MH_GEMM_DMA", "MH_GEMM_PP", "MH_DMA_STAGGER")))
        self.tile_report = None
        self.warm_passes = 0
        self.warm_passes_run = 0
        self.aux_flag = hip.AUX_U8 if os.environ.get("MAESTRO_AUX_U8", "1") == "1" else 0
        self._tuned = set()
        gc.collect()
        if os.environ.get("MAESTRO_KEEP_RETIRED_GRAPHS", "0") != "1":
            drain_retired_graphs()
        self._graphs, self._seen, self._ready_spans = {}, {}, []
        weakref.finalize(self, _retire_graphs, self._graphs)
        self._inputs = {}
        prio = int(os.environ.get("MAESTRO_SIDE_PRIORITY", "0"))
        self.side_streams = [torch.cuda.Stream(device=device, priority=prio) for _ in range(max(0, n_side_streams))]
        self._wgrad_stream = torch.cuda.Stream(device=device)
        self._wgrad_tables = {}
        self._dw_conv_clear = False

    def _stable_inputs(self, batch: dict) -> dict:
        out = {}
        for k, t in batch.items():
            if not isinstance(t, torch.Tensor) or not t.is_cuda:
                out[k] = t
                continue
            st = self._inputs.get(k)
            if st is None:
                self._inputs[k] = {"ptr": t.data_ptr(), "buf": None}
                out[k] = t
            elif st["buf"] is None and st["ptr"] == t.data_ptr():
                out[k] = t
            else:
                buf = st["buf"]
                if buf is None or buf.shape != t.shape or buf.dtype != t.dtype:
                    buf = st["buf"] = torch.empty_like(t, memory_format=torch.contiguous_format)
                if buf.data_ptr() != t.data_ptr():
                    buf.copy_(t)
                out[k] = buf
        return out

    def _alloc_embed(self) -> None:
        self.embed = {name: PatchEmbedEnd(self, s) for name, s in self.mods.items()}
        self.mb = {name: end.buf for name, end in self.embed.items()}

    def _pack_conv_weights(self) -> None:
        for end in self.embed.values():
            end.pack()

    def _stage_inputs(self, batch: dict) -> dict:
        sources = [parts[0] for parts in self.model.src_specs.values()]
        for s in sources:
            img = batch[s.src]
            if img.dtype != F32 or not img.is_contiguous() or not img.is_cuda:
                raise ValueError(f"batch[{s.src!r}] must be a contiguous float32 GPU tensor")
            d = batch[f"{s.src}_dates"]
            if d.dtype != torch.int16 or not d.is_contiguous():
                raise ValueError(f"batch['{s.src}_dates'] must be a contiguous int16 tensor [B, D, 3]")
        batch = self._stable_inputs(batch)
        for s in sources:
            img = batch[s.src]
            if tuple(img.shape[-2:]) != (s.S, s.S) or self.model.interpolate != "nearest":
                mode = {"nearest": 0, "bilinear": 1, "bicubic": 2}.get(self.model.interpolate)
                if mode is None:
                    raise ValueError(f"Invalid interpolate mode {self.model.interpolate!r} (nearest, bilinear, bicubic)")
                buf = self.mb[s.name].get("resized")
                if buf is None:
                    buf = self.mb[s.name]["resized"] = torch.empty(self.B, s.Dates, s.C_src, s.S, s.S, dtype=F32, device=self.device)
                hip.resize(img, buf, self.B * s.Dates * s.C_src, img.shape[-2], img.shape[-1], s.S, s.S, mode)
                batch[s.src] = buf
        self._staged = batch
        self._cur_key = tuple(batch[k].data_ptr() for k in sorted(batch) if isinstance(batch[k], torch.Tensor))
        return batch

    def returned_batch(self, batch: dict) -> dict:
        out = dict(batch)
        sources = [parts[0] for parts in self.model.src_specs.values()]
        out.update({s.src: self._staged[s.src] for s in sources})
        for s in sources:
            if s.rescale_elev:
                img = out[s.src]
                res = torch.empty_like(img)
                hip.rescale_elev(img, res, img.shape[0] * img.shape[1], s.C_src, s.S)
                out[s.src] = res
        return out

    def _grads_ready(self, module) -> None:
        ps = list(module.parameters())
        if ps:
            self._ready_spans.append(self.store.span(ps))

    def _run_parallel(self, fns) -> None:
        if len(fns) == 1 or not self.multi_stream or not self.group_streams:
            for fn in fns:
                fn()
            return
        main = torch.cuda.current_stream()
        sides = self.side_streams[: len(fns) - 1]
        for side in sides:
            side.wait_stream(main)
        fns[0]()
        for side, fn in zip(sides, fns[1:]):
            with torch.cuda.stream(side):
                fn()
        for side in sides:
            main.wait_stream(side)

    def _instep_tune(self, one_pass) -> None:
        self.instep_tune = False
        if (getattr(self, "fp8", None) is not None or getattr(self, "_opt", None) is not None or hip.kernel_timer_active()
                or torch.cuda.is_current_stream_capturing()):
            return
        saved = (self.use_graphs, self.multi_stream, self.grad_hook)
        self.use_graphs, self.multi_stream, self.grad_hook = False, False, None
        tuner = hip.InStepTuner()
        hip.set_instep_tuner(tuner)
        try:
            one_pass()
            for cand in tuner.CANDIDATES:
                tuner.begin(cand)
                one_pass()
            tuner.begin(None)
            self.tile_report = tuner.finish()
        finally:
            hip.set_instep_tuner(None)
            self.use_graphs, self.multi_stream, self.grad_hook = saved

    def _warm_up(self, one_pass) -> None:
        global _PROCESS_WARMED
        n, self.warm_passes = self.warm_passes, 0
        self.warm_passes_run = 0
        if (n <= 0 or _PROCESS_WARMED or getattr(self, "fp8", None) is not None or getattr(self, "_opt", None) is not None
                or hip.kernel_timer_active() or torch.cuda.is_current_stream_capturing() or not torch.is_grad_enabled()):
            return
        _PROCESS_WARMED = True
        hook, graphs = self.grad_hook, self.use_graphs
        self.use_graphs = False
        if hook is not None:
            self.grad_hook = lambda lo, hi: None
        try:
            for _ in range(n):
                one_pass()
                self.warm_passes_run += 1
        finally:
            self.grad_hook, self.use_graphs = hook, graphs

    def _first_step_passes(self, one_pass) -> None:
        if self.instep_tune:
            self._instep_tune(one_pass)
        if self.warm_passes > 0:
            self._warm_up(one_pass)

    def _launch_wgrads(self, items, ends=()) -> None:
        items = [(st, lo, hi) for st, lo, hi in items if hi > lo]
        if not items and not ends:
            return
        key = (tuple((st.tag, lo, hi) for st, lo, hi in items), tuple(ends))
        table = self._wgrad_tables.get(key)
        if table is None:
            if torch.cuda.is_current_stream_capturing():
                raise hip.HipExtensionError(f"weight-gradient table {key} first needed inside a hipGraph capture")
            probs = [p for st, lo, hi in items for p in st.wgrad_problems(lo, hi)]
            jobs = [j for st, lo, hi in items for j in st.reduce_jobs(lo, hi)]
            after, ready = [], []
            for tag in ends:
                e_probs, e_jobs, e_after, e_ready = self._ends_table(tag)
                probs, jobs, after, ready = probs + e_probs, jobs + e_jobs, after + e_after, ready + e_ready
            table = self._wgrad_tables[key] = (hip.GroupedTN(probs, self.device) if probs else None,
                                               hip.ColsumBatch(jobs, self.device) if jobs else None, after, ready)
        if table[1] is not None:
            table[1].launch()
        if table[0] is not None:
            table[0].launch()
        for fn in table[2]:
            fn()
        for module in table[3]:
            self._grads_ready(module)

    @contextlib.contextmanager
    def _tuning_pass(self, what: str):
        if not self.tune_gemm or what in self._tuned or hip.kernel_timer_active():
            yield
            return
        saved = self.multi_stream
        self.multi_stream = False
        hip.set_gemm_tuning(True)
        try:
            yield
        finally:
            hip.set_gemm_tuning(False)
            self.multi_stream = saved
            self._tuned.add(what)

    def _segment(self, name: str, key, fn) -> None:
        if _ROCTX:
            torch.cuda.nvtx.range_push(f"maestro:{name.split(':')[0]}")
            try:
                return self._segment_run(name, key, fn)
            finally:
                torch.cuda.nvtx.range_pop()
        return self._segment_run(name, key, fn)

    def _segment_run(self, name: str, key, fn) -> None:
        if not self.use_graphs or hip.kernel_timer_active():
            self._ready_spans = []
            fn()
            self._flush_ready(self._ready_spans)
            return
        entry = self._graphs.get(name)
        if entry is not None and entry["key"] == key:
            entry["graph"].replay()
            self._flush_ready(entry["spans"])
            return
        seen = self._seen.get(name, _NEVER)
        self._ready_spans = []
        if seen == key:
            graph = torch.cuda.CUDAGraph()
            gc_was_on, failure = gc.isenabled(), None
            gc.disable()
            try:
                with torch.cuda.graph(graph, capture_error_mode="thread_local"):
                    fn()
            except Exception as exc:
                failure = exc
            finally:
                if gc_was_on:
                    gc.enable()
            if failure is not None:
                import warnings
                warnings.warn(f"hipGraph capture of segment {name!r} failed ({failure}); continuing with eager launches")
                self.use_graphs = False
                torch.cuda.synchronize()
                self._ready_spans = []
                fn()
                self._flush_ready(self._ready_spans)
                return
            self._graphs[name] = {"key": key, "graph": graph, "spans": list(self._ready_spans)}
            graph.replay()
        else:
            self._seen[name] = key
            fn()
        self._flush_ready(self._ready_spans)

    def _flush_ready(self, spans) -> None:
        if self.grad_hook is not None:
            for lo, hi in spans:
                self.grad_hook(lo, hi)



class MAEEngine(EngineBase):
    def __init__(self, model, batch_size: int, device, loss: str = "l2_norm", dtype: str = "bf16",
                 fp8_scaling: str | None = None, deterministic: bool = False) -> None:
        self.deterministic = bool(deterministic)
        if self.deterministic and dtype == "fp8":
            raise ValueError("deterministic=True is not available with dtype='fp8' (the amax / scale bookkeeping is not covered)")
        if loss not in ("l1", "l2", "l1_norm", "l2_norm"):
            raise ValueError(f"Invalid loss {loss}.")
        if dtype not in ("bf16", "fp8"):
            raise ValueError(f"Invalid compute dtype {dtype!r} (bf16, fp8)")
        scaling = resolve_scaling(fp8_scaling)
        self.fp8_scaling = scaling if dtype == "fp8" else None
        device = torch.device(device)
        if device.type != "cuda":
            raise hip.HipExtensionError("MAEEngine needs a GPU device; the MAE hot path has no CPU fallback")
        hip.lib()
        self.model, self.B, self.device, self.loss, self.dtype = model, batch_size, device, loss, dtype
        self.fp8, self._fp8_weights = None, {}
        self.p_loss = 1 if loss.startswith("l1") else 2
        self.normalise = loss.endswith("_norm")
        m = model
        self.e2d_identity = m.embed_dim == m.decoder_dim
        self.E, self.Dd = m.embed_dim, m.decoder_dim
        self._init_runtime(device, len(model.group_specs) - 1)
        self.wgrad_mode = os.environ.get("MAESTRO_WGRAD", "auto")
        if self.wgrad_mode not in ("auto", "fused", "deferred"):
            raise ValueError(f"MAESTRO_WGRAD={self.wgrad_mode!r}: expected auto, fused or deferred")
        self._wgrad_plans, self._zero_lists = {}, {}
        self.ends_parts = frozenset(os.environ.get("MAESTRO_ENDS", "abc")) if not self.deterministic and dtype != "fp8" else frozenset()
        if not self.ends_parts <= frozenset("abc") or ("c" in self.ends_parts and "b" not in self.ends_parts):
            raise ValueError(f"MAESTRO_ENDS={os.environ.get('MAESTRO_ENDS')!r}: a subset of 'abc' expected, 'c' only with 'b'")
        self._loss_cs = False
        self._ends_ws = {}
        self._det_sites, self._det_tables = {"fwd": {}, "bwd": {}}, {}
        self._h2d_done = [None] * RING
        self._opt = None
        self.host_wait_s = 0.0
        self._step = 0
        self._enc_state = {}
        B = batch_size
        fold = m.fusion_mode in ("shared", "monotemp")
        self.mods, self.groups = m.mod_specs, list(m.group_specs.values())
        for s in self.mods.values():
            s.Beff = B * s.Dates if fold else B
        for g in self.groups:
            g.Beff = g.mods[0].Beff
        ordered = []
        for name in m.patch_embed:
            ordered += [(f"patch_embed.{name}.{k}", p) for k, p in m.patch_embed[name].named_parameters()]
        for name in m.encoder:
            ordered += [(f"encoder.{name}.{k}", p) for k, p in m.encoder[name].named_parameters()]
        if m.encoder_inter is not None:
            ordered += [(f"encoder_inter.{k}", p) for k, p in m.encoder_inter.named_parameters()]
        for name in m.enc_to_dec:
            ordered += [(f"enc_to_dec.{name}.{k}", p) for k, p in m.enc_to_dec[name].named_parameters()]
        ordered += [(f"mask_token.{k}", p) for k, p in m.mask_token.items()]
# ... 902 lines not shown
```

### maestro_amd/hip.py

```python

from __future__ import annotations

import contextlib
import ctypes
import os
from pathlib import Path

import torch

_LIB_PATH = Path(__file__).resolve().parent / "lib" / "libmaestro_hip.so"
_lib = None

GEMM_NT, GEMM_NN, GEMM_TN = 0, 1, 2
OUT_F32, BIAS, GELU, RESIDUAL, DGELU, ATOMIC, COLSUM, AUX_DGELU, MULAUX, C8_E5M2, AUX_U8 = 1, 2, 4, 8, 16, 32, 64, 128, 256, 512, 1024


class HipExtensionError(RuntimeError):
    pass


def lib() -> ctypes.CDLL:
    global _lib
    if _lib is None:
        if not _LIB_PATH.exists():
            raise HipExtensionError(
                f"{_LIB_PATH} not found: build it with `python -m maestro_amd.csrc.build` "
                "(or __graft_entry__.build()).  The MAE hot path has no fallback implementation.")
        retired = [v for v in ("MAESTRO_GROUPED", "MH_GEMM_SPLITK", "MH_ATTN_BWD", "MAESTRO_CU_MASK") if os.environ.get(v)]
        if retired:
            raise HipExtensionError(f"{', '.join(retired)}: retired experiment switch(es) -- the variant no longer exists, this run "
                                    "would measure the default path (INTEGRATION.md, profiles/r05_experiments.md, r06_experiments.md)")
        _lib = ctypes.CDLL(str(_LIB_PATH))
        _lib.mh_last_error.restype = ctypes.c_char_p
        _lib.mh_layernorm_bwd_workspace.restype = _lib.mh_gemm_sk_workspace.restype = ctypes.c_long
        _lib.mh_attn_reduce_partial_rows.restype = ctypes.c_long
        vp, ci = ctypes.c_void_p, ctypes.c_int
        _lib.mh_confusion_ce.argtypes = [vp, vp, ci, ctypes.c_long, vp, ci, ci, ci, ci, ci, vp]
        _lib.mh_confusion_bce.argtypes = [vp, vp, ctypes.c_float, ctypes.c_float, vp, ci, ci, vp]
        _lib.mh_confusion_ce.restype = _lib.mh_confusion_bce.restype = ci
        _lib.mh_reduce_ordered.argtypes = [vp, vp, ci, vp, ci, vp]
        _lib.mh_colsum_partial_rows.argtypes = [ci]
        _lib.mh_masked_loss_partial_size.argtypes = _lib.mh_embed_bwd_partial_rows.argtypes = [ci, ci]
        _lib.mh_unmask_token_grad_partial_rows.argtypes = [ctypes.c_long]
        _lib.mh_masked_loss_cs_rows.argtypes = [ci, ci]
        _lib.mh_gather_rows_cs_rows.argtypes = _lib.mh_embed_bwd_cs_rows.argtypes = [ctypes.c_long]
        _lib.mh_select_dates.argtypes = [vp, ci, vp, ci, ci, vp, vp, vp, ci, vp, vp, vp, vp, ci, ci, ci, ctypes.c_long, ci, ci,
                                         ctypes.c_float, vp]
        _lib.mh_select_dates.restype = ci
    return _lib


def _check(rc: int, what: str) -> None:
    if rc != 0:
        msg = lib().mh_last_error().decode(errors="replace")
        raise HipExtensionError(f"{what} failed (rc={rc}): {msg}")


def ptr(t: torch.Tensor | None):
    if t is None:
        return ctypes.c_void_p(0)
    if not t.is_cuda:
        raise HipExtensionError("maestro_amd kernels need GPU tensors (no CPU fallback)")
    return ctypes.c_void_p(t.data_ptr())


def stream():
    return ctypes.c_void_p(torch.cuda.current_stream().cuda_stream)


_I, _F, _L = ctypes.c_int, ctypes.c_float, ctypes.c_long


TILE_AUTO, TILE_REG_128, TILE_DMA_256, TILE_DMA_256x128, TILE_DMA_128x256, TILE_DMA_128, TILE_DMA_128x4 = -1, 0, 1, 2, 3, 4, 5
TILE_DMA_256_LOCKSTEP = 6
TILE_REG_64, TILE_REG_192 = 13, 14
TILE_SK_192, TILE_SK_256, TILE_SK_DMA_256 = 15, 16, 17
SK_TILES = (TILE_SK_192, TILE_SK_256, TILE_SK_DMA_256)
TILE_PP_128 = 7
TILES = (TILE_REG_128, TILE_DMA_256, TILE_DMA_256x128, TILE_DMA_128x256, TILE_DMA_128, TILE_DMA_128x4)
_LAYOUT_NAME = {0: "NT", 1: "NN", 2: "TN"}
_TILE_NAME = {TILE_REG_128: "gemm_kernel<{}>", TILE_DMA_256: "gemm_dma_kernel<256x256,{}>",
              TILE_DMA_256x128: "gemm_dma_kernel<256x128,{}>", TILE_DMA_128x256: "gemm_dma_kernel<128x256,{}>",
              TILE_DMA_128: "gemm_dma_kernel<128x128,{}>", TILE_DMA_128x4: "gemm_dma_kernel<128x128q,{}>",
              TILE_DMA_256_LOCKSTEP: "gemm_dma_kernel<256x256,{}>", TILE_PP_128: "gemm_pp_kernel<{}>",
              TILE_REG_64: "gemm_kernel<{},64x128>", TILE_REG_192: "gemm_kernel<{},192x128>",
              TILE_SK_192: "gemm_sk_kernel<{},192x128>", TILE_SK_256: "gemm_sk_kernel<{},256x128>",
              TILE_SK_DMA_256: "gemm_sk_dma_kernel<256x256,{}>"}
_tile_choice: dict = {}
_tuning = False


def set_gemm_tuning(on: bool) -> None:
    global _tuning
    _tuning = bool(on)


def gemm_tile_choices() -> dict:
    return dict(_tile_choice)


class InStepTuner:

    CANDIDATES = (TILE_AUTO, TILE_REG_128, TILE_PP_128, TILE_REG_64, TILE_REG_192, TILE_DMA_256) + (
        (TILE_SK_DMA_256, TILE_SK_192, TILE_SK_256) if os.environ.get("MAESTRO_INSTEP_SK") == "1" else ())

    def __init__(self) -> None:
        self.cand, self.ev, self.bad = None, {}, set()

    def begin(self, cand) -> None:
        self.cand = cand

    def open(self, key):
        e0, e1 = torch.cuda.Event(enable_timing=True), torch.cuda.Event(enable_timing=True)
        self.ev.setdefault(key, {}).setdefault(self.cand, []).append((e0, e1))
        return e0, e1

    def reject(self, key) -> None:
        self.bad.add((key, self.cand))

    def finish(self, margin: float = 0.03) -> dict:
        torch.cuda.synchronize()
        report = {}
        for key, per in self.ev.items():
            base_n = len(per.get(TILE_AUTO, ()))
            ms = {c: sum(a.elapsed_time(b) for a, b in evs) for c, evs in per.items()
                  if (key, c) not in self.bad and len(evs) == base_n and base_n}
            if TILE_AUTO not in ms:
                continue
            best = min(ms, key=ms.get)
            pick = best if ms[best] < (1.0 - margin) * ms[TILE_AUTO] else TILE_AUTO
            _tile_choice[key] = pick
            report[key] = (pick, ms)
        return report


_instep: InStepTuner | None = None


def set_instep_tuner(t: InStepTuner | None) -> None:
    global _instep
    _instep = t


_sk_ws: dict = {}
_sk_grid = None


def sk_grid() -> int:
    global _sk_grid
    if _sk_grid is None:
        env = os.environ.get("MH_SK_GRID")
        _sk_grid = int(env) if env else torch.cuda.get_device_properties(torch.cuda.current_device()).multi_processor_count
    return _sk_grid


def sk_workspace(tile: int, grid: int) -> torch.Tensor:
    key = (torch.cuda.current_stream().cuda_stream, tile, grid)
    ws = _sk_ws.get(key)
    if ws is None:
        nbytes = lib().mh_gemm_sk_workspace(_I(tile), _I(grid))
        if nbytes <= 0:
            raise HipExtensionError(f"mh_gemm_sk_workspace({tile}, {grid}) = {nbytes}")
        if torch.cuda.is_current_stream_capturing():
            raise HipExtensionError("stream-K workspace requested for the first time inside a hipGraph capture: run the step eagerly once first")
        ws = torch.zeros(nbytes, dtype=torch.uint8, device="cuda")
        _sk_ws[key] = ws
    return ws


def sk_error_flag(ws: torch.Tensor) -> int:
    return int(ws[4092:4096].view(torch.int32).item())


def gemm_sk(tile: int, layout: int, M: int, N: int, K: int, A, lda: int, B, ldb: int, C, ldc: int, flags: int = 0, bias=None,
            res=None, ldr: int = 0, grid: int | None = None) -> int:
    grid = grid or sk_grid()
    ws = sk_workspace(tile, grid)
    return lib().mh_gemm_bf16_sk(_I(tile), _I(layout), _I(M), _I(N), _I(K), ptr(A), _I(lda), ptr(B), _I(ldb), ptr(C), _I(ldc),
                                 _I(flags), ptr(bias), ptr(res), _I(ldr), ptr(ws), _L(ws.numel()), _I(grid), stream())


def _gemm_tile(tile, layout, M, N, K, A, lda, B, ldb, C, ldc, flags, bias, res, ldr, aux_in, aux_out, ldaux, colsum) -> int:
    if tile in SK_TILES:
        return gemm_sk(tile, layout, M, N, K, A, lda, B, ldb, C, ldc, flags, bias, res, ldr)
    return lib().mh_gemm_bf16_tile(_I(tile), _I(layout), _I(M), _I(N), _I(K), ptr(A), _I(lda), ptr(B), _I(ldb), ptr(C),
                                   _I(ldc), _I(flags), ptr(bias), ptr(res), _I(ldr), ptr(aux_in), ptr(aux_out), _I(ldaux),
                                   ptr(colsum), stream())


FAMILY_DMA, FAMILY_PP, FAMILY_192, FAMILY_ALL = 1, 2, 4, 7


def resolve_tile(tile, layout, M, N, K, lda, ldb, ldc, ldr, ldaux, flags, families=FAMILY_ALL) -> int:
    rc = lib().mh_gemm_bf16_resolve_tile(_I(tile), _I(families), _I(layout), _I(M), _I(N), _I(K), _I(lda), _I(ldb), _I(ldc), _I(ldr),
                                         _I(ldaux), _I(flags))
    if rc == -1:
        _check(rc, "mh_gemm_bf16_resolve_tile")
    return rc


def _resolve(tile, args, families=FAMILY_ALL) -> int:
    layout, M, N, K, _, lda, _, ldb, _, ldc, flags, _, _, ldr, _, _, ldaux, _ = args
    return resolve_tile(tile, layout, M, N, K, lda, ldb, ldc, ldr, ldaux, flags, families)


def _tune_gemm(key, args) -> int:
    best, best_ms = TILE_REG_128, float("inf")
    for tile in TILES:
        rc = _gemm_tile(tile, *args)
        if rc == -2:
            continue
        _check(rc, "mh_gemm_bf16_tile")
        _gemm_tile(tile, *args)
        e0, e1 = torch.cuda.Event(enable_timing=True), torch.cuda.Event(enable_timing=True)
        e0.record()
        for _ in range(4):
            _gemm_tile(tile, *args)
        e1.record()
        e1.synchronize()
        ms = e0.elapsed_time(e1)
        if ms < best_ms:
            best, best_ms = tile, ms
    _tile_choice[key] = best
    return best


_shape_only = 0


@contextlib.contextmanager
def shape_only_tiles():
    global _shape_only
    _shape_only += 1
    try:
        yield
    finally:
        _shape_only -= 1


def _pick_tile(layout, M, N, K, flags, args) -> int:
    if _shape_only:
        return TILE_AUTO
    tflags = flags & ~COLSUM
    key = (layout, M, N, K, tflags)
    tile = _tile_choice.get(key)
    if tile is None:
        forced = os.environ.get("MH_GEMM_TILE")
        if forced is not None:
            t = int(forced)
            if TILE_PP_128 < t <= TILE_PP_128 + 5 and os.environ.get("MH_ALLOW_DIAG_TILES") != "1":
                raise HipExtensionError(f"MH_GEMM_TILE={t} selects a diagnostic build of the ping-pong tile that writes wrong "
                                        "outputs (present only in a -DMH_DIAG_TILES library); set MH_ALLOW_DIAG_TILES=1 to run it on purpose")
            return t
        dma = os.environ.get("MH_GEMM_DMA", "")[:1]
        if os.environ.get("MH_GEMM_PP", "")[:1] == "0" and dma == "":
            return _resolve(TILE_AUTO, args, FAMILY_DMA)
        if dma == "0":
            return TILE_REG_128
        lockstep = os.environ.get("MH_DMA_STAGGER", "")[:1] == "0"
        if (dma == "1" and layout != GEMM_TN and not (flags & ATOMIC)) or (
                lockstep and _resolve(TILE_AUTO, args, FAMILY_DMA) == TILE_DMA_256):
            return TILE_DMA_256_LOCKSTEP if lockstep else TILE_DMA_256
        if _tuning and not (flags & ATOMIC):
            targs = list(args)
            targs[10], targs[17] = tflags, None
            tile = _tune_gemm(key, tuple(targs))
        else:
            tile = TILE_AUTO
    return tile


def gemm(layout: int, M: int, N: int, K: int, A, lda: int, B, ldb: int, C, ldc: int, flags: int = 0, bias=None,
         res=None, ldr: int = 0, aux_in=None, aux_out=None, ldaux: int = 0, colsum=None, tile: int | None = None) -> None:
    args = (layout, M, N, K, A, lda, B, ldb, C, ldc, flags, bias, res, ldr, aux_in, aux_out, ldaux, colsum)
    explicit = tile is not None
    if _instep is not None and _instep.cand is not None and not explicit and not (flags & ATOMIC):
        key = (layout, M, N, K, flags & ~COLSUM)
        e0, e1 = _instep.open(key)
        e0.record()
        rc = _gemm_tile(_instep.cand, *args)
        if rc == -2:
            _instep.reject(key)
            rc = _gemm_tile(TILE_AUTO, *args)
        _check(rc, "mh_gemm_bf16_tile")
        e1.record()
        return
    if not explicit:
        tile = _pick_tile(layout, M, N, K, flags, args)
    ev = None
    if _timer is not None:
        named = tile if tile in SK_TILES else _resolve(tile, args)
        if named == -2:
            named = tile
        ev = _timer.record(_TILE_NAME[named].format(_LAYOUT_NAME[layout]), 2.0 * M * N * K, (M, N, K))
        ev[0].record()
    rc = _gemm_tile(tile, *args)
    if rc == -2 and not explicit:
        pinned = os.environ.get("MH_GEMM_DMA", "")[:1] == "1" or os.environ.get("MH_GEMM_PP", "")[:1] == "0"
        rc = _gemm_tile(TILE_REG_128 if pinned else TILE_AUTO, *args)
    if rc == -2:
        raise HipExtensionError(f"mh_gemm_bf16_tile: problem ({M}, {N}, {K}) does not qualify for tile {tile}")
    _check(rc, "mh_gemm_bf16_tile")
    if ev is not None:
        ev[1].record()


def call(name: str, *args) -> None:
    conv = []
    for a in args:
        if a is None or isinstance(a, torch.Tensor):
            conv.append(ptr(a))
        else:
            conv.append(a)
    _check(getattr(lib(), name)(*conv, stream()), name)


def _hbm_call(kind: str, nbytes: float, name: str, *args) -> None:
    if _timer is None:
        return call(name, *args)
    e0, e1 = _timer.record_bytes(kind, nbytes)
    e0.record()
    call(name, *args)
    e1.record()


def _esz(t) -> int:
    return 0 if t is None else t.element_size()


def layernorm_fwd(x, x_L, x_off, gamma, beta, y, y_L, y_off, mean, rstd, B, n, dim, eps=1e-5):
    _hbm_call(f"ln_fwd<{dim}>", float(B) * n * dim * (4 + _esz(y)), "mh_layernorm_fwd", x, _I(x_L), _I(x_off), gamma, beta, y, _I(y_L),
              _I(y_off), _I(1 if y.dtype == torch.float32 else 0), mean, rstd, _I(B), _I(n), _I(dim), _F(eps))


def layernorm_fwd_fp8(x, x_L, x_off, gamma, beta, y, y_L, y_off, mean, rstd, B, n, dim, y8, y8_scale, y8_amax, eps=1e-5):
    call("mh_layernorm_fwd_fp8", x, _I(x_L), _I(x_off), gamma, beta, y, _I(y_L), _I(y_off), mean, rstd, _I(B), _I(n), _I(dim),
         _F(eps), y8, y8_scale, y8_amax)


def layernorm_fwd_mx(x, x_L, x_off, gamma, beta, y, y_L, y_off, mean, rstd, B, n, dim, y8, y8_scales, ld_y8s, eps=1e-5):
    call("mh_layernorm_fwd_mx", x, _I(x_L), _I(x_off), gamma, beta, y, _I(y_L), _I(y_off), mean, rstd, _I(B), _I(n), _I(dim),
         _F(eps), y8, y8_scales, _I(ld_y8s))


def layernorm_bwd_workspace(rows, dim) -> int:
    return int(lib().mh_layernorm_bwd_workspace(_I(rows), _I(dim)))


def layernorm_bwd(dy, dy_L, dy_off, x, x_L, x_off, gamma, mean, rstd, dres, dx, dx_bf16, dgamma, dbeta, dcol, workspace,
                  B, n, dim):
    _hbm_call(f"ln_bwd<{dim}>", float(B) * n * dim * (_esz(dy) + 4 + _esz(dres) + 4 + _esz(dx_bf16)), "mh_layernorm_bwd", dy, _I(dy_L),
              _I(dy_off), _I(1 if dy.dtype == torch.float32 else 0), x, _I(x_L), _I(x_off), gamma, mean, rstd, dres, dx, dx_bf16,
              dgamma, dbeta, dcol, workspace, _I(B), _I(n), _I(dim))


def layernorm_bwd_partial(dy, dy_L, dy_off, x, x_L, x_off, gamma, mean, rstd, dres, dx, dx_bf16, workspace, B, n, dim):
    _hbm_call(f"ln_bwd<{dim}>", float(B) * n * dim * (_esz(dy) + 4 + _esz(dres) + 4 + _esz(dx_bf16)), "mh_layernorm_bwd_partial", dy,
              _I(dy_L), _I(dy_off), _I(1 if dy.dtype == torch.float32 else 0), x, _I(x_L), _I(x_off), gamma, mean, rstd, dres, dx,
              dx_bf16, workspace, _I(B), _I(n), _I(dim))


COLSUM_ROWS = 16


class _MhColsumJob(ctypes.Structure):
    _fields_ = [("src", ctypes.c_void_p), ("dst", ctypes.c_void_p), ("rows", ctypes.c_int), ("cols", ctypes.c_int),
                ("ld", ctypes.c_int), ("reserved", ctypes.c_int)]


class ColsumBatch:

    def __init__(self, jobs, device) -> None:
        if not jobs:
            raise HipExtensionError("ColsumBatch: no jobs")
        arr = (_MhColsumJob * len(jobs))()
        for i, (src, dst, rows, cols, ld) in enumerate(jobs):
            if src.dtype != torch.float32 or dst.dtype != torch.float32 or not src.is_cuda or not dst.is_cuda:
                raise HipExtensionError("ColsumBatch: f32 device tensors expected")
            if rows <= 0 or cols <= 0 or ld < cols or src.numel() < (rows - 1) * ld + cols or dst.numel() < cols:
                raise HipExtensionError(f"ColsumBatch job {i}: shape ({rows}, {cols}, ld {ld}) does not fit its buffers")
            arr[i] = _MhColsumJob(src.data_ptr(), dst.data_ptr(), rows, cols, ld, 0)
        self.keep = [t for job in jobs for t in job[:2]]
        self.table = torch.frombuffer(bytearray(bytes(arr)), dtype=torch.uint8).to(device)
        blocks = []
        for i, (_, _, rows, cols, _) in enumerate(jobs):
            if cols > 65535 * 256 or len(jobs) > 32767:
                raise HipExtensionError("ColsumBatch: too many jobs / columns for the work-item encoding")
            for cb in range(-(-cols // 256)):
                blocks += [(i << 48) | (cb << 32) | rc for rc in range(-(-rows // COLSUM_ROWS))]
        self.blocks = torch.tensor(blocks, dtype=torch.int64).to(device)
        self.n, self.n_blocks = len(jobs), len(blocks)

    def launch(self) -> None:
        call("mh_colsum_batched", self.table, _I(self.n), self.blocks, _I(self.n_blocks))


ORDERED_ROWS, ORDERED_ADD = 16, 1
COLSUM_PARTIAL_ROWS = 256


class _MhOrderedJob(ctypes.Structure):
    _fields_ = [("src", ctypes.c_void_p), ("dst", ctypes.c_void_p), ("rows", ctypes.c_int), ("cols", ctypes.c_int),
                ("ld", ctypes.c_int), ("flags", ctypes.c_int)]


class OrderedReduce:

    def __init__(self, jobs, device) -> None:
        if not jobs:
            raise HipExtensionError("OrderedReduce: no jobs")
        chains: dict = {}
        for i, job in enumerate(jobs):
            if len(job) not in (5, 6):
                raise HipExtensionError(f"OrderedReduce job {i}: (src, dst, rows, cols, ld[, add]) expected")
            src, dst, rows, cols, ld = job[:5]
            add = bool(job[5]) if len(job) == 6 else False
            if not (isinstance(src, torch.Tensor) and isinstance(dst, torch.Tensor)) or src.dtype != torch.float32 \
                    or dst.dtype != torch.float32 or not src.is_cuda or not dst.is_cuda:
                raise HipExtensionError(f"OrderedReduce job {i}: f32 device tensors expected")
            if rows <= 0 or cols <= 0 or ld < cols or src.numel() < (rows - 1) * ld + cols or dst.numel() < cols:
                raise HipExtensionError(f"OrderedReduce job {i}: shape ({rows}, {cols}, ld {ld}) does not fit its buffers")
            chain = chains.setdefault(dst.data_ptr(), [])
            if chain and (chain[0][3] != cols or chain[0][5] != add):
                raise HipExtensionError(f"OrderedReduce job {i}: cols / add differ from the other jobs of its destination")
            chain.append((src, dst, rows, cols, ld, add))
        spans = sorted((c[0][1].data_ptr(), c[0][1].data_ptr() + 4 * c[0][3]) for c in chains.values())
        if any(a[1] > b[0] for a, b in zip(spans, spans[1:])):
            raise HipExtensionError("OrderedReduce: two destinations overlap without being the same")
        flat = [j for chain in chains.values() for j in chain]
        arr = (_MhOrderedJob * len(flat))()
        blocks, i = [], 0
        for chain in chains.values():
            blocks += [(i << 32) | cb for cb in range(-(-chain[0][3] // 256))]
            for src, dst, rows, cols, ld, add in chain:
                arr[i] = _MhOrderedJob(src.data_ptr(), dst.data_ptr(), rows, cols, ld, ORDERED_ADD if add else 0)
                i += 1
        self.keep = [t for j in flat for t in j[:2]]
        self.host = arr
        self.table = torch.frombuffer(bytearray(bytes(arr)), dtype=torch.uint8).to(device)
        self.blocks = torch.tensor(blocks, dtype=torch.int64).to(device)
        self.n, self.n_blocks, self.n_chains = len(flat), len(blocks), len(chains)
        self.nbytes = 4.0 * (sum(j[2] * j[3] for j in flat) + sum(c[0][3] for c in chains.values()))

    def launch(self) -> None:
        ev = _timer.record_bytes("reduce_ordered", self.nbytes) if _timer is not None else None
        if ev is not None:
            ev[0].record()
        _check(lib().mh_reduce_ordered(ctypes.byref(self.host), ptr(self.table), _I(self.n), ptr(self.blocks), _I(self.n_blocks),
                                       stream()), "mh_reduce_ordered")
        if ev is not None:
            ev[1].record()


def colsum_partial_rows(M) -> int:
    return int(lib().mh_colsum_partial_rows(_I(M)))


def colsum_partial(x, partial, M, N, ld):
    call("mh_colsum_partial", x, _I(1 if x.dtype == torch.float32 else 0), partial, _I(M), _I(N), _I(ld))


def masked_loss_partial_size(B, Lm) -> int:
    return int(lib().mh_masked_loss_partial_size(_I(B), _I(Lm)))


def masked_loss_det(rec, target, mask_group, n_masked, weight, loss_partial, drec, B, Lm, Lgroup, tok_off, PPC, p):
    _hbm_call("masked_loss", float(B) * Lm * (PPC * (_esz(rec) + 4 + _esz(drec)) + 1), "mh_masked_loss_det", rec, target, mask_group,
              n_masked, _F(weight), loss_partial, drec, _I(B), _I(Lm), _I(Lgroup), _I(tok_off), _I(PPC), _I(p))


def masked_loss_bands_det(rec, target, mask_group, n_elems, weight, loss_partial, drec, B, Lm, Lgroup, tok_off, PPC, p, tgt_C,
                          tgt_c0, n_g):
    call("mh_masked_loss_bands_det", rec, target, mask_group, n_elems, _F(weight), loss_partial, drec, _I(B), _I(Lm), _I(Lgroup),
         _I(tok_off), _I(PPC), _I(p), _I(tgt_C), _I(tgt_c0), _I(n_g))


def unmask_token_grad_partial_rows(n_rows) -> int:
    return int(lib().mh_unmask_token_grad_partial_rows(_L(n_rows)))


def unmask_token_grad_det(dxdec, mask, tok_slot, partial, B, L, Dd, slot, t_lo, t_hi):
    call("mh_unmask_token_grad_det", dxdec, mask, tok_slot, partial, _I(B), _I(L), _I(Dd), _I(slot), _I(t_lo), _I(t_hi))


def unmask_token_grad_per_sample_det(dxdec, mask, tok_slot_bl, partial, B, L, Dd, slot):
    call("mh_unmask_token_grad_per_sample_det", dxdec, mask, tok_slot_bl, partial, _I(B), _I(L), _I(Dd), _I(slot))


def embed_bwd_partial_rows(BD, L) -> int:
    return int(lib().mh_embed_bwd_partial_rows(_I(BD), _I(L)))


def embed_finish_bwd_det(dxg, y, stats, gamma, dyc, param_partial, blk_sums, sums, B, D, L, E, tok_off, Lgroup):
    call("mh_embed_finish_bwd_det", dxg, y, stats, gamma, dyc, param_partial, blk_sums, sums, _I(B), _I(D), _I(L), _I(E),
         _I(tok_off), _I(Lgroup))


def masked_loss_cs_rows(B, Lm) -> int:
    return int(lib().mh_masked_loss_cs_rows(_I(B), _I(Lm)))


def masked_loss_cs(rec, target, mask_group, n_masked, weight, acc, drec, cs_partial, B, Lm, Lgroup, tok_off, PPC, p):
    _hbm_call("masked_loss", float(B) * Lm * (PPC * (_esz(rec) + 4 + _esz(drec)) + 1), "mh_masked_loss_cs", rec, target, mask_group,
              n_masked, _F(weight), acc, drec, cs_partial, _I(B), _I(Lm), _I(Lgroup), _I(tok_off), _I(PPC), _I(p))


def masked_loss_bands_cs(rec, target, mask_group, n_elems, weight, acc, drec, cs_partial, B, Lm, Lgroup, tok_off, PPC, p, tgt_C,
                         tgt_c0, n_g):
    call("mh_masked_loss_bands_cs", rec, target, mask_group, n_elems, _F(weight), acc, drec, cs_partial, _I(B), _I(Lm), _I(Lgroup),
         _I(tok_off), _I(PPC), _I(p), _I(tgt_C), _I(tgt_c0), _I(n_g))


def gather_rows_cs_rows(rows) -> int:
    return int(lib().mh_gather_rows_cs_rows(_L(rows)))


def gather_rows_bf16_cs(src, idx, dst16, cs_partial, B, src_L, n_idx, dim):
    call("mh_gather_rows_bf16_cs", src, idx, dst16, cs_partial, _I(B), _I(src_L), _I(n_idx), _I(dim))


def embed_bwd_cs_rows(rows) -> int:
    return int(lib().mh_embed_bwd_cs_rows(_L(rows)))


def embed_finish_bwd_ends(dx, inv, n_vis, y, stats, gamma, dyc, dgamma, dbeta, sums, cs_partial, B, D, L, E, tok_off, Lgroup):
    call("mh_embed_finish_bwd_ends", dx, inv, _I(n_vis), y, stats, gamma, dyc, dgamma, dbeta, sums, cs_partial, _I(B), _I(D), _I(L),
         _I(E), _I(tok_off), _I(Lgroup))


def det_slices(K: int) -> int:
    return max(1, min(8, K // 1024))


def gemm_tn_slabs(M, N, K, A, lda, B, ldb, slabs):
    S = slabs.shape[0]
    step = -(-(-(-K // S)) // 64) * 64
    for i in range(S):
        k0 = i * step
        kn = min(K, k0 + step) - k0
        if kn <= 0:
            raise HipExtensionError(f"gemm_tn_slabs: empty K-slice {i} of {S} (K = {K})")
        gemm(GEMM_TN, M, N, kn, A[k0:], lda, B[k0:], ldb, slabs[i], N, OUT_F32)


def attn_fwd(qkv, out, lse, B, N, H, D, scale):
    call("mh_attn_fwd", qkv, out, lse, _I(B), _I(N), _I(H), _I(D), _F(scale))


def attn_bwd(qkv, out, dout, lse, delta, dqkv, B, N, H, D, scale):
    call("mh_attn_bwd", qkv, out, dout, lse, delta, dqkv, _I(B), _I(N), _I(H), _I(D), _F(scale))


def patchify(img, cols, target, BD, Ctot, S, P, Kpad, norm_bands, n_groups, normalise, rescale_elev):
    nb = float(BD) * S * S * Ctot * 4 + float(BD) * (S // P) ** 2 * (Kpad * 2 * (cols is not None) + Ctot * P * P * 4 * (target is not None))
    _hbm_call("patchify", nb, "mh_patchify", img, cols, target, _I(BD), _I(Ctot), _I(S), _I(P), _I(Kpad), norm_bands, _I(n_groups),
              _I(int(normalise)), _I(int(rescale_elev)))


def patchify_bands(img, cols, target, BD, Csrc, c0, Ctot, S, P, Kpad, norm_bands, n_groups, normalise, rescale_elev):
    call("mh_patchify_bands", img, cols, target, _I(BD), _I(Csrc), _I(c0), _I(Ctot), _I(S), _I(P), _I(Kpad), norm_bands,
         _I(n_groups), _I(int(normalise)), _I(int(rescale_elev)))


def groupnorm_partial_size(BD, L, E) -> int:
    return int(lib().mh_groupnorm_partial_size(_I(BD), _I(L), _I(E)))


def groupnorm_stats(y, partial, stats, BD, L, E, eps=1e-5):
    call("mh_groupnorm_stats", y, partial, stats, _I(BD), _I(L), _I(E), _F(eps))


def embed_finish(y, stats, gamma, beta, pos, date, date_rows, date_off, xg, B, D, L, E, tok_off, Lgroup):
    call("mh_embed_finish", y, stats, gamma, beta, pos, date, _I(date_rows), _I(date_off), xg, _I(B), _I(D), _I(L), _I(E),
         _I(tok_off), _I(Lgroup))


def date_features(dates, ref_date, out, B, D, rows, row_off, fac):
    call("mh_date_features", dates, ref_date, out, _I(B), _I(D), _I(rows), _I(row_off), _F(fac))


def resize(src, dst, planes, Hin, Win, Hout, Wout, mode):
    call("mh_resize", src, dst, _L(planes), _I(Hin), _I(Win), _I(Hout), _I(Wout), _I(mode))


def rescale_elev(img, out, BD, C, S):
    call("mh_rescale_elev", img, out, _I(BD), _I(C), _I(S))


def embed_finish_bwd(dxg, y, stats, gamma, dyc, dgamma, dbeta, sums, B, D, L, E, tok_off, Lgroup):
    call("mh_embed_finish_bwd", dxg, y, stats, gamma, dyc, dgamma, dbeta, sums, _I(B), _I(D), _I(L), _I(E), _I(tok_off),
         _I(Lgroup))
# ... 580 lines not shown
```

Before: 1863.

## Use register-direct accumulator epilogue forms in the 256x256 DMA GEMM kernel

Moves the pipelined kernel's direct-from-accumulator epilogue (bf16, GELU with u8 aux, mul-aux with colsum, f32 bias+residual) into a shared EpiAcc header. The 256x256 DMA kernel now uses it by default when the flags and alignments qualify. This skips the LDS staging round-trip and the trailing barrier of the generic epilogue, storing straight from registers with buffer stores. It adds more kernel instantiations and a new colsum reduction path based on DPP row sums. MH_DMA_EPI=0 restores the old behaviour.

```diff
diff --git a/include/maestro_hip.h b/include/maestro_hip.h
--- a/include/maestro_hip.h
+++ b/include/maestro_hip.h
@@ -33,7 +33,8 @@
        MH_TILE_PP_128_DIAG4 = 11, MH_TILE_PP_128_DIAG5 = 12,
        MH_TILE_REG_64 = 13, MH_TILE_REG_192 = 14,
        MH_TILE_SK_192 = 15, MH_TILE_SK_256 = 16,
-       MH_TILE_SK_DMA_256 = 17  };
+       MH_TILE_SK_DMA_256 = 17,
+       MH_TILE_DMA_256_EPI0 = 18, MH_TILE_DMA_256_LOCKSTEP_EPI0 = 19 };
 int mh_gemm_bf16_tile(int tile, int layout, int M, int N, int K, const void* A, int lda, const void* B, int ldb, void* C,
                       int ldc, int flags, const float* bias, const float* res, int ldr, const void* aux_in, void* aux_out,
                       int ldaux, float* colsum, void* stream);
diff --git a/maestro_amd/csrc/gemm.hip b/maestro_amd/csrc/gemm.hip
--- a/maestro_amd/csrc/gemm.hip
+++ b/maestro_amd/csrc/gemm.hip
@@ -194,10 +194,14 @@
     return 0;
 }
 
+static bool is_dma_tile(int tile) {
+    return (tile > MH_TILE_REG_128 && tile < MH_TILE_PP_128) || tile == MH_TILE_DMA_256_EPI0 || tile == MH_TILE_DMA_256_LOCKSTEP_EPI0;
+}
+
 static int gemm_check_args(bool buffers, int tile, int layout, const GemmParams& p) {
     const int M = p.M, N = p.N, K = p.K, lda = p.lda, ldb = p.ldb, ldc = p.ldc, ldr = p.ldr, ldaux = p.ldaux, flags = p.flags;
     auto given = [&](const void* q) { return !buffers || q; };
-    MH_CHECK_ARG(tile >= MH_TILE_AUTO && tile <= MH_TILE_REG_192, "mh_gemm_bf16: tile %d", tile);
+    MH_CHECK_ARG((tile >= MH_TILE_AUTO && tile <= MH_TILE_REG_192) || is_dma_tile(tile), "mh_gemm_bf16: tile %d", tile);
     MH_CHECK_ARG(layout >= 0 && layout <= 2, "mh_gemm_bf16: layout %d", layout);
     MH_CHECK_ARG(!(flags & ~0x7ff), "mh_gemm_bf16: unknown flag bits 0x%x", flags & ~0x7ff);
     MH_CHECK_ARG(M > 0 && N > 0 && K > 0, "mh_gemm_bf16: empty problem %d %d %d", M, N, K);
@@ -240,7 +244,7 @@
 static int gemm_resolve(int tile, int families, int layout, const GemmParams& p) {
     const int M = p.M, N = p.N, K = p.K, flags = p.flags;
     if (tile >= MH_TILE_PP_128 && tile <= MH_TILE_PP_128_DIAG5) return gemm_pp_serves(tile, layout, p) ? tile : -2;
-    if (tile > MH_TILE_REG_128 && tile < MH_TILE_PP_128) return gemm_dma_serves(tile, layout, p) ? tile : -2;
+    if (is_dma_tile(tile)) return gemm_dma_serves(tile, layout, p) ? tile : -2;
     if (tile != MH_TILE_AUTO)
         return layout != 2 && !(flags & MH_GEMM_COLSUM) ? tile : MH_TILE_REG_128;
     const bool dma = (families & MH_GEMM_FAMILY_DMA) && prefer_dma(layout, M, N, K, flags);
@@ -273,7 +277,7 @@
     const int run = gemm_resolve(tile, MH_GEMM_FAMILY_ALL, layout, p);
     if (run == -2) return -2;
     if (run >= MH_TILE_PP_128 && run <= MH_TILE_PP_128_DIAG5) return gemm_pp_launch(run, layout, p, (hipStream_t)stream);
-    if (run > MH_TILE_REG_128 && run < MH_TILE_PP_128) return gemm_dma_launch(run, layout, p, (hipStream_t)stream);
+    if (is_dma_tile(run)) return gemm_dma_launch(run, layout, p, (hipStream_t)stream);
     return gemm_reg_launch(run, layout, p, (hipStream_t)stream);
 }
 
diff --git a/maestro_amd/csrc/gemm_dma.hip b/maestro_amd/csrc/gemm_dma.hip
--- a/maestro_amd/csrc/gemm_dma.hip
+++ b/maestro_amd/csrc/gemm_dma.hip
@@ -1,4 +1,5 @@
 #include "gemm_ring.hpp"
+#include "gemm_epi_acc.hpp"
 
 #ifndef MH_DMA_PRIO
 #define MH_DMA_PRIO 0
@@ -13,7 +14,7 @@
 
 namespace {
 
-template <class T, bool A_KMAJOR, bool B_KMAJOR, int CALLER, bool STAGGER>
+template <class T, bool A_KMAJOR, bool B_KMAJOR, int CALLER, bool STAGGER, int EPI = EPI_GENERIC>
 __device__ __forceinline__ void gemm_dma_tile(const GemmParams& p, int tile_m, int tile_n, int kbeg, int kend,
                                               unsigned char* smem) {
     constexpr int S = T::S, PA = T::PA, PB = T::PB, NW = T::NW;
@@ -119,15 +120,19 @@
             load_step(t);
             math_step();
         }
-        __builtin_amdgcn_s_barrier();
-    }
-
-    float* st = reinterpret_cast<float*>(smem) + w * (32 * 68);
-    if (p.flags & MH_GEMM_ATOMIC) gemm_epilogue_atomic<MT>(p, acc, st, m0 + wm, n0 + wn);
-    else gemm_epilogue_store<MT>(p, acc, st, m0 + wm, n0 + wn);
-}
-
-template <class T, bool A_KMAJOR, bool B_KMAJOR, bool STAGGER>
+        if constexpr (EPI == EPI_GENERIC) __builtin_amdgcn_s_barrier();
+    }
+
+    if constexpr (EPI == EPI_GENERIC) {
+        float* st = reinterpret_cast<float*>(smem) + w * (32 * 68);
+        if (p.flags & MH_GEMM_ATOMIC) gemm_epilogue_atomic<MT>(p, acc, st, m0 + wm, n0 + wn);
+        else gemm_epilogue_store<MT>(p, acc, st, m0 + wm, n0 + wn);
+    } else {
+        if (n0 + wn < p.N && m0 + wm < p.M) epi_acc_exposed<EPI, MT, T::WN>(p, acc, m0, n0, w);
+    }
+}
+
+template <class T, bool A_KMAJOR, bool B_KMAJOR, bool STAGGER, int EPI = EPI_GENERIC>
 __global__ __launch_bounds__(T::NT, T::MIN_WG) void gemm_dma_kernel(GemmParams p) {
     __shared__ __attribute__((aligned(16))) unsigned char smem[T::LDS_BYTES];
     const int nwg = p.tiles_m * p.tiles_n;
@@ -135,7 +140,7 @@
     int tile_m, tile_n;
     raster_tile<4>(p, id, tile_m, tile_n);
     const int kbeg = blockIdx.y * p.k_per_split;
-    gemm_dma_tile<T, A_KMAJOR, B_KMAJOR, 0, STAGGER>(p, tile_m, tile_n, kbeg, min(p.K, kbeg + p.k_per_split), smem);
+    gemm_dma_tile<T, A_KMAJOR, B_KMAJOR, 0, STAGGER, EPI>(p, tile_m, tile_n, kbeg, min(p.K, kbeg + p.k_per_split), smem);
 }
 
 typedef Tile<2, 4, 4> T256;
@@ -164,8 +169,40 @@
     gemm_dma_tile<T, true, true, 1, STAGGER>(p, tile_m, tile_n, 0, g.K, smem);
 }
 
+constexpr unsigned DMA_EPI_FORMS = (1u << EPI_BF16) | (1u << EPI_GELU) | (1u << EPI_MULAUX) | (1u << EPI_F32);
+int dma_epilogue_form(int layout, const GemmParams& p) {
+    const int epi = epi_acc_form(p.flags);
+    if (epi < 0 || !((DMA_EPI_FORMS >> epi) & 1u) || layout == 2 || p.N % 64 != 0) return EPI_GENERIC;
+    if (p.c8 || p.descale_a || p.descale_b || p.sa || p.sb) return EPI_GENERIC;
+    const long rows = (long)ceil_div(p.M, 256) * 256;
+    if (epi == EPI_F32) {
+        if (p.ldc % 4 != 0 || p.ldr % 4 != 0 || !gemm_in_reach(rows * p.ldc * 4) || !gemm_in_reach(rows * p.ldr * 4)) return EPI_GENERIC;
+    } else {
+        if (p.ldc % 8 != 0 || !gemm_in_reach(rows * p.ldc * 2)) return EPI_GENERIC;
+        if (epi != EPI_BF16 && (p.ldaux % 8 != 0 || !gemm_in_reach(rows * p.ldaux))) return EPI_GENERIC;
+        if (epi == EPI_MULAUX && (long)ceil_div(p.M, 64) * p.N * 4 >= (1L << 29)) return EPI_GENERIC;
+    }
+    return epi;
+}
+
+template <class T, bool STAGGER>
+void launch_dma_epi(int epi, int layout, const GemmParams& p, dim3 grid, dim3 block, hipStream_t s) {
+#define MH_DMA_EPI_CASE(E)                                                                                        \
+    case E:                                                                                                       \
+        if (layout == 0) hipLaunchKernelGGL((gemm_dma_kernel<T, false, false, STAGGER, E>), grid, block, 0, s, p); \
+        else hipLaunchKernelGGL((gemm_dma_kernel<T, false, true, STAGGER, E>), grid, block, 0, s, p);              \
+        break;
+    switch (epi) {
+        MH_DMA_EPI_CASE(EPI_BF16)
+        MH_DMA_EPI_CASE(EPI_GELU)
+        MH_DMA_EPI_CASE(EPI_MULAUX)
+        default: MH_DMA_EPI_CASE(EPI_F32)
+    }
+#undef MH_DMA_EPI_CASE
+}
+
 template <class T>
-void launch_dma(int layout, GemmParams& p, hipStream_t s, bool stagger = true) {
+void launch_dma(int layout, GemmParams& p, hipStream_t s, bool stagger = true, bool epi_forms = false) {
     const int K = p.K;
     p.tiles_m = ceil_div(p.M, T::BM); p.tiles_n = ceil_div(p.N, T::BN);
     int splits = 1;
@@ -178,6 +215,14 @@
     p.k_per_split = ksteps_per * BK;
     splits = ceil_div(K, p.k_per_split);
     dim3 grid(p.tiles_m * p.tiles_n, splits), block(T::NT);
+    if constexpr (T::BM == 256 && T::BN == 256) {
+        const int epi = epi_forms ? dma_epilogue_form(layout, p) : EPI_GENERIC;
+        if (epi != EPI_GENERIC) {
+            if (stagger) launch_dma_epi<T, true>(epi, layout, p, grid, block, s);
+            else launch_dma_epi<T, false>(epi, layout, p, grid, block, s);
+            return;
+        }
+    }
     if (T::NW == 8 && stagger) {
         switch (layout) {
             case 0: hipLaunchKernelGGL((gemm_dma_kernel<T, false, false, T::NW == 8>), grid, block, 0, s, p); break;
@@ -208,7 +253,8 @@
 bool gemm_dma_serves(int tile, int layout, const GemmParams& p) {
     int bm, bn;
     switch (tile) {
-        case MH_TILE_DMA_256: case MH_TILE_DMA_256_LOCKSTEP: bm = T256::BM; bn = T256::BN; break;
+        case MH_TILE_DMA_256: case MH_TILE_DMA_256_LOCKSTEP: case MH_TILE_DMA_256_EPI0: case MH_TILE_DMA_256_LOCKSTEP_EPI0:
+            bm = T256::BM; bn = T256::BN; break;
         case MH_TILE_DMA_256x128: bm = T256x128::BM; bn = T256x128::BN; break;
         case MH_TILE_DMA_128x256: bm = T128x256::BM; bn = T128x256::BN; break;
         case MH_TILE_DMA_128: case MH_TILE_DMA_128x4: bm = T128::BM; bn = T128::BN; break;
@@ -225,12 +271,14 @@
     p.fast = 1;
     gemm_set_extents(p, layout);
     switch (tile) {
-        case MH_TILE_DMA_256: launch_dma<T256>(layout, p, s); break;
+        case MH_TILE_DMA_256: launch_dma<T256>(layout, p, s, true, true); break;
+        case MH_TILE_DMA_256_EPI0: launch_dma<T256>(layout, p, s, true, false); break;
+        case MH_TILE_DMA_256_LOCKSTEP_EPI0: launch_dma<T256>(layout, p, s, false, false); break;
         case MH_TILE_DMA_256x128: launch_dma<T256x128>(layout, p, s); break;
         case MH_TILE_DMA_128x256: launch_dma<T128x256>(layout, p, s); break;
         case MH_TILE_DMA_128: launch_dma<T128>(layout, p, s); break;
         case MH_TILE_DMA_128x4: launch_dma<T128q>(layout, p, s); break;
-        default: launch_dma<T256>(layout, p, s, false); break;
+        default: launch_dma<T256>(layout, p, s, false, true); break;
     }
     MH_LAUNCH_CHECK();
     return 0;
diff --git a/maestro_amd/csrc/gemm_epi_acc.hpp b/maestro_amd/csrc/gemm_epi_acc.hpp
--- /dev/null
+++ b/maestro_amd/csrc/gemm_epi_acc.hpp
@@ -0,0 +1,237 @@
+#pragma once
+#include "gemm_common.hpp"
+#include <type_traits>
+
+namespace {
+
+enum { EPI_GENERIC = -1, EPI_BF16 = 0, EPI_GELU = 1, EPI_MULAUX = 2, EPI_F32 = 3 };
+
+inline int epi_acc_form(int flags) {
+    if (flags == 0) return EPI_BF16;
+    if (flags == (MH_GEMM_BIAS | MH_GEMM_GELU | MH_GEMM_AUX_DGELU | MH_GEMM_AUX_U8)) return EPI_GELU;
+    if (flags == (MH_GEMM_MULAUX | MH_GEMM_AUX_U8 | MH_GEMM_COLSUM)) return EPI_MULAUX;
+    if (flags == (MH_GEMM_OUT_F32 | MH_GEMM_BIAS | MH_GEMM_RESIDUAL)) return EPI_F32;
+    return -1;
+}
+
+__device__ __forceinline__ void swap16(uint32_t& a, uint32_t& b) {
+    const u32x2 r = __builtin_amdgcn_permlane16_swap(a, b, false, false);
+    a = r[0]; b = r[1];
+}
+
+__device__ __forceinline__ float row16_sum(float v) {
+#define MH_ROW_ROR(n) __builtin_bit_cast(float, __builtin_amdgcn_update_dpp(0, __builtin_bit_cast(int, v), 0x120 + (n), 0xf, 0xf, false))
+    v += MH_ROW_ROR(8);
+    v += MH_ROW_ROR(4);
+    v += MH_ROW_ROR(2);
+    v += MH_ROW_ROR(1);
+#undef MH_ROW_ROR
+    return v;
+}
+
+template <int EPI, int MT, int DIAG = 0, bool EXPOSED = false>
+struct EpiAcc {
+    static constexpr int CS_DROP = 1 << 30;
+    static constexpr int CHUNKS = 2 * MT;
+    const GemmParams& p;
+    const __amdgpu_buffer_rsrc_t rc_dst, raux, rbias, rcs;
+    int e_c = 0, e_aux = 0, e_bias = 0, e_cs = 0;
+    f32x4 bias_x = {0, 0, 0, 0}, bias_y = {0, 0, 0, 0};
+    f32x4 cs_x[2] = {{0, 0, 0, 0}, {0, 0, 0, 0}}, cs_y[2] = {{0, 0, 0, 0}, {0, 0, 0, 0}};
+    u32x4 ld_x = {0, 0, 0, 0}, ld_y = {0, 0, 0, 0};
+
+    __device__ __forceinline__ explicit EpiAcc(const GemmParams& p_)
+        : p(p_),
+          rc_dst(__builtin_amdgcn_make_buffer_rsrc(
+              p_.C, (short)0, (int)(((long)(p_.M - 1) * p_.ldc + p_.N) * (EPI == EPI_F32 ? 4 : 2)), 0x00020000)),
+          raux(__builtin_amdgcn_make_buffer_rsrc(
+              EPI == EPI_GELU ? (void*)p_.aux_out : EPI == EPI_MULAUX ? (void*)p_.aux_in : (void*)p_.res, (short)0,
+              (int)(EPI == EPI_F32 ? ((long)(p_.M - 1) * p_.ldr + p_.N) * 4 : EPI == EPI_BF16 ? 0 : (long)(p_.M - 1) * p_.ldaux + p_.N), 0x00020000)),
+          rbias(__builtin_amdgcn_make_buffer_rsrc((void*)p_.bias, (short)0, p_.bias ? p_.N * 4 : 0, 0x00020000)),
+          rcs(__builtin_amdgcn_make_buffer_rsrc(
+              (void*)p_.colsum, (short)0, EPI == EPI_MULAUX ? (int)((long)((p_.M + 63) / 64) * p_.N * 4) : 0, 0x00020000)) {}
+
+    template <int WN>
+    __device__ __forceinline__ void setup(int m0, int n0, int w) {
+        int lane = __builtin_amdgcn_mbcnt_hi(~0u, __builtin_amdgcn_mbcnt_lo(~0u, 0u));
+        asm volatile("" : "+v"(lane));
+        const int g = lane >> 4, lm = lane & 15;
+        const int wm = (w / WN) * (16 * MT), wn = (w % WN) * 64;
+        const int col_nat = wn + 4 * g;
+        const int col_swp = wn + 4 * g + 12 * (g & 1);
+        const int row = m0 + wm + lm;
+        if constexpr (EPI == EPI_F32) {
+            e_c = (row * p.ldc + n0 + col_nat) * 4;
+            e_aux = (row * p.ldr + n0 + col_nat) * 4;
+        } else {
+            e_c = (row * p.ldc + n0 + col_swp) * 2;
+            e_aux = row * p.ldaux + n0 + (EPI == EPI_GELU || EXPOSED ? col_swp : col_nat);
+        }
+        e_bias = (n0 + col_nat) * 4;
+        e_cs = (((m0 + wm) >> 6) * p.N + n0 + col_nat) * 4;
+        if constexpr (EXPOSED) e_cs = lm == 0 ? e_cs : CS_DROP;
+    }
+
+    template <int jp>
+    __device__ __forceinline__ void load_bias() {
+        bias_x = __builtin_bit_cast(f32x4, __builtin_amdgcn_raw_buffer_load_b128(rbias, e_bias + 128 * jp, 0, 0));
+        bias_y = __builtin_bit_cast(f32x4, __builtin_amdgcn_raw_buffer_load_b128(rbias, e_bias + 128 * jp + 64, 0, 0));
+    }
+
+    template <class CC>
+    __device__ __forceinline__ void loads(CC) {
+        constexpr int c = CC::value, jp = c / MT, i = c % MT;
+        if constexpr (DIAG == 1) return;
+        if constexpr ((EPI == EPI_GELU || EPI == EPI_F32) && !EXPOSED) {
+            if constexpr (i == 0) load_bias<jp>();
+        }
+        if constexpr (EPI == EPI_F32) {
+            const int o = e_aux + (16 * i * p.ldr + 32 * jp) * 4;
+            ld_x = __builtin_amdgcn_raw_buffer_load_b128(raux, o, 0, 0);
+            ld_y = __builtin_amdgcn_raw_buffer_load_b128(raux, o + 64, 0, 0);
+        }
+        if constexpr (EPI == EPI_MULAUX) {
+            const int o = e_aux + 16 * i * p.ldaux + 32 * jp;
+            if constexpr (EXPOSED) {
+                const u32x2 b8 = __builtin_amdgcn_raw_buffer_load_b64(raux, o, 0, 0);
+                ld_x[0] = b8[0]; ld_y[0] = b8[1];
+            } else {
+                ld_x[0] = __builtin_amdgcn_raw_buffer_load_b32(raux, o, 0, 0);
+                ld_y[0] = __builtin_amdgcn_raw_buffer_load_b32(raux, o + 16, 0, 0);
+            }
+        }
+    }
+
+    template <class CC>
+    __device__ __forceinline__ void math(CC, const f32x4 (&src)[4][MT]) {
+        constexpr int c = CC::value, jp = c / MT, i = c % MT;
+        f32x4 vx = src[2 * jp][i], vy = src[2 * jp + 1][i];
+        if constexpr (DIAG == 1) {
+            asm volatile("" ::"v"(vx), "v"(vy));
+            return;
+        }
+        if constexpr (EPI == EPI_F32) {
+            const int o = e_c + (16 * i * p.ldc + 32 * jp) * 4;
+            vx = vx + (bias_x + __builtin_bit_cast(f32x4, ld_x));
+            vy = vy + (bias_y + __builtin_bit_cast(f32x4, ld_y));
+            __builtin_amdgcn_raw_buffer_store_b128(__builtin_bit_cast(u32x4, vx), rc_dst, o, 0, 0);
+            __builtin_amdgcn_raw_buffer_store_b128(__builtin_bit_cast(u32x4, vy), rc_dst, o + 64, 0, 0);
+            return;
+        } else {
+            if constexpr (EPI == EPI_GELU) {
+                vx += bias_x; vy += bias_y;
+                f32x4 cx, dx, cy, dy;
+                if constexpr (DIAG == 3) { cx = vx; dx = vx; cy = vy; dy = vy; }
+                else { gelu_cdf_pdf4(vx, cx, dx); gelu_cdf_pdf4(vy, cy, dy); }
+                const f32x4 gx = vx * dx + cx, gy = vy * dy + cy;
+                uint32_t bx = 0, by = 0;
+#pragma unroll
+                for (int e = 0; e < 4; ++e) {
+                    bx = __builtin_amdgcn_cvt_pk_u8_f32(__builtin_fmaf(gx[e], 200.f, 26.f), e, bx);
+                    by = __builtin_amdgcn_cvt_pk_u8_f32(__builtin_fmaf(gy[e], 200.f, 26.f), e, by);
+                }
+                swap16(bx, by);
+                if constexpr (DIAG == 2) asm volatile("" ::"v"(bx), "v"(by));
+                else __builtin_amdgcn_raw_buffer_store_b64((u32x2){bx, by}, raux, e_aux + 16 * i * p.ldaux + 32 * jp, 0, 0);
+                vx *= cx; vy *= cy;
+            }
+            if constexpr (EPI == EPI_MULAUX) {
+                constexpr int s = EXPOSED ? jp : 0;
+                f32x4 &sx = cs_x[s], &sy = cs_y[s];
+                uint32_t ax = ld_x[0], ay = ld_y[0];
+                if constexpr (EXPOSED) swap16(ax, ay);
+                vx *= unpack_dgelu_u8x4(ax);
+                vy *= unpack_dgelu_u8x4(ay);
+                if constexpr (i % 4 == 0) { sx = vx; sy = vy; } else { sx += vx; sy += vy; }
+                if constexpr (i % 4 == 3) {
+                    if constexpr (EXPOSED) {
+#pragma unroll
+                        for (int e = 0; e < 4; ++e) { sx[e] = row16_sum(sx[e]); sy[e] = row16_sum(sy[e]); }
+                    } else {
+#pragma unroll
+                        for (int o = 1; o < 16; o <<= 1) {
+#pragma unroll
+                            for (int e = 0; e < 4; ++e) {
+                                sx[e] += __shfl_xor(sx[e], o, 64);
+                                sy[e] += __shfl_xor(sy[e], o, 64);
+                            }
+                        }
+                    }
+                    const int o_cs = e_cs + (i / 4) * p.N * 4 + 128 * jp;
+                    __builtin_amdgcn_raw_buffer_store_b128(__builtin_bit_cast(u32x4, sx), rcs, o_cs, 0, 0);
+                    __builtin_amdgcn_raw_buffer_store_b128(__builtin_bit_cast(u32x4, sy), rcs, o_cs + 64, 0, 0);
+                }
+            }
+            uint32_t x0 = pack_bf2(vx[0], vx[1]), x1 = pack_bf2(vx[2], vx[3]);
+            uint32_t y0 = pack_bf2(vy[0], vy[1]), y1 = pack_bf2(vy[2], vy[3]);
+            swap16(x0, y0);
+            swap16(x1, y1);
+            if constexpr (DIAG == 2) asm volatile("" ::"v"(x0), "v"(x1), "v"(y0), "v"(y1));
+            else __builtin_amdgcn_raw_buffer_store_b128((u32x4){x0, x1, y0, y1}, rc_dst, e_c + (16 * i * p.ldc + 32 * jp) * 2, 0, 0);
+        }
+    }
+};
+
+template <int B, int E, class F>
+__device__ __forceinline__ void epi_for(F&& f) {
+    if constexpr (B < E) {
+        f(std::integral_constant<int, B>{});
+        epi_for<B + 1, E>(f);
+    }
+}
+
+template <int EPI, int MT, int WN>
+__device__ __forceinline__ void epi_acc_exposed(const GemmParams& p, const f32x4 (&acc)[4][MT], int m0, int n0, int w) {
+    constexpr int NC = 2 * MT, BATCH = 4, NB = NC / BATCH;
+    static_assert(MT % BATCH == 0, "a batch of residual loads stays inside one column pair");
+    auto ord = [](int k) constexpr { return EPI == EPI_F32 ? k : (k % 2) * MT + k / 2; };
+    EpiAcc<EPI, MT, 0, true> e(p);
+    e.template setup<WN>(m0, n0, w);
+    f32x4 tbx[2], tby[2];
+    uint32_t ax[NC], ay[NC];
+    u32x4 tx[2][BATCH], ty[2][BATCH];
+    if constexpr (EPI == EPI_GELU || EPI == EPI_F32) {
+        epi_for<0, 2>([&](auto jj) {
+            constexpr int jp = decltype(jj)::value;
+            e.template load_bias<jp>();
+            tbx[jp] = e.bias_x; tby[jp] = e.bias_y;
+        });
+    }
+    if constexpr (EPI == EPI_MULAUX) {
+        epi_for<0, NC>([&](auto kk) {
+            constexpr int c = ord(decltype(kk)::value);
+            e.loads(std::integral_constant<int, c>{});
+            ax[c] = e.ld_x[0]; ay[c] = e.ld_y[0];
+        });
+    }
+    if constexpr (EPI == EPI_F32) {
+        auto fetch = [&](auto bb) {
+            constexpr int b = decltype(bb)::value;
+            epi_for<0, BATCH>([&](auto kk) {
+                constexpr int k = decltype(kk)::value;
+                e.loads(std::integral_constant<int, b * BATCH + k>{});
+                tx[b & 1][k] = e.ld_x; ty[b & 1][k] = e.ld_y;
+            });
+        };
+        fetch(std::integral_constant<int, 0>{});
+        epi_for<0, NB>([&](auto bb) {
+            constexpr int b = decltype(bb)::value;
+            if constexpr (b + 1 < NB) fetch(std::integral_constant<int, b + 1>{});
+            epi_for<0, BATCH>([&](auto kk) {
+                constexpr int k = decltype(kk)::value, c = b * BATCH + k;
+                e.ld_x = tx[b & 1][k]; e.ld_y = ty[b & 1][k];
+                e.bias_x = tbx[c / MT]; e.bias_y = tby[c / MT];
+                e.math(std::integral_constant<int, c>{}, acc);
+            });
+        });
+    } else {
+        epi_for<0, NC>([&](auto kk) {
+            constexpr int c = ord(decltype(kk)::value);
+            if constexpr (EPI == EPI_GELU) { e.bias_x = tbx[c / MT]; e.bias_y = tby[c / MT]; }
+            if constexpr (EPI == EPI_MULAUX) { e.ld_x[0] = ax[c]; e.ld_y[0] = ay[c]; }
+            e.math(std::integral_constant<int, c>{}, acc);
+        });
+    }
+}
+
+}
diff --git a/maestro_amd/csrc/gemm_pp.hip b/maestro_amd/csrc/gemm_pp.hip
--- a/maestro_amd/csrc/gemm_pp.hip
+++ b/maestro_amd/csrc/gemm_pp.hip
@@ -1,4 +1,5 @@
 #include "gemm_reg.hpp"
+#include "gemm_epi_acc.hpp"
 #include <type_traits>
 
 #ifndef MH_PP_PRIO
@@ -7,13 +8,7 @@
 
 namespace {
 
-enum { EPI_BF16 = 0, EPI_GELU = 1, EPI_MULAUX = 2, EPI_F32 = 3 };
 constexpr int EPI_STEPS = 8;
-
-__device__ __forceinline__ void swap16(uint32_t& a, uint32_t& b) {
-    const u32x2 r = __builtin_amdgcn_permlane16_swap(a, b, false, false);
-    a = r[0]; b = r[1];
-}
 
 template <bool B_KMAJOR, int EPI, int DIAG = 0>
 __global__ __launch_bounds__(NT, 2) void gemm_pp_kernel(GemmParams p) {
@@ -64,114 +59,11 @@
     f32x4 acc[4][4], prev[4][4];
     int sidx = 0;
 
-    const __amdgpu_buffer_rsrc_t rc_dst = __builtin_amdgcn_make_buffer_rsrc(
-        p.C, (short)0, (int)(((long)(p.M - 1) * p.ldc + p.N) * (EPI == EPI_F32 ? 4 : 2)), 0x00020000);
-    const __amdgpu_buffer_rsrc_t raux = __builtin_amdgcn_make_buffer_rsrc(
-        EPI == EPI_GELU ? (void*)p.aux_out : EPI == EPI_MULAUX ? (void*)p.aux_in : (void*)p.res, (short)0,
-        (int)(EPI == EPI_F32 ? ((long)(p.M - 1) * p.ldr + p.N) * 4 : EPI == EPI_BF16 ? 0 : (long)(p.M - 1) * p.ldaux + p.N), 0x00020000);
-    const __amdgpu_buffer_rsrc_t rbias = __builtin_amdgcn_make_buffer_rsrc((void*)p.bias, (short)0, p.bias ? p.N * 4 : 0, 0x00020000);
-    const __amdgpu_buffer_rsrc_t rcs = __builtin_amdgcn_make_buffer_rsrc(
-        (void*)p.colsum, (short)0, EPI == EPI_MULAUX ? (int)((long)((p.M + 63) / 64) * p.N * 4) : 0, 0x00020000);
     const int w_s = __builtin_amdgcn_readfirstlane(w);
-    int e_c = 0, e_aux = 0, e_bias = 0, e_cs = 0;
-    f32x4 bias_x = {0, 0, 0, 0}, bias_y = {0, 0, 0, 0};
-    f32x4 cs_x = {0, 0, 0, 0}, cs_y = {0, 0, 0, 0};
-    u32x4 ld_x = {0, 0, 0, 0}, ld_y = {0, 0, 0, 0};
-    auto epi_setup = [&](int m0, int n0) {
-        int lane = __builtin_amdgcn_mbcnt_hi(~0u, __builtin_amdgcn_mbcnt_lo(~0u, 0u));
-        asm volatile("" : "+v"(lane));
-        const int g = lane >> 4, lm = lane & 15;
-        const int wm = (w_s >> 1) * 64, wn = (w_s & 1) * 64;
-        const int col_nat = wn + 4 * g;
-        const int col_swp = wn + 4 * g + 12 * (g & 1);
-        const int row = m0 + wm + lm;
-        if constexpr (EPI == EPI_F32) {
-            e_c = (row * p.ldc + n0 + col_nat) * 4;
-            e_aux = (row * p.ldr + n0 + col_nat) * 4;
-        } else {
-            e_c = (row * p.ldc + n0 + col_swp) * 2;
-            e_aux = row * p.ldaux + n0 + (EPI == EPI_GELU ? col_swp : col_nat);
-        }
-        e_bias = (n0 + col_nat) * 4;
-        e_cs = (((m0 + wm) >> 6) * p.N + n0 + col_nat) * 4;
-    };
-    auto epi_loads = [&](auto cc) {
-        constexpr int c = decltype(cc)::value, jp = c >> 2, i = c & 3;
-        if constexpr (DIAG == 1) return;
-        if constexpr (EPI == EPI_GELU || EPI == EPI_F32) {
-            if constexpr (i == 0) {
-                bias_x = __builtin_bit_cast(f32x4, __builtin_amdgcn_raw_buffer_load_b128(rbias, e_bias + 128 * jp, 0, 0));
-                bias_y = __builtin_bit_cast(f32x4, __builtin_amdgcn_raw_buffer_load_b128(rbias, e_bias + 128 * jp + 64, 0, 0));
-            }
-        }
-        if constexpr (EPI == EPI_F32) {
-            const int o = e_aux + (16 * i * p.ldr + 32 * jp) * 4;
-            ld_x = __builtin_amdgcn_raw_buffer_load_b128(raux, o, 0, 0);
-            ld_y = __builtin_amdgcn_raw_buffer_load_b128(raux, o + 64, 0, 0);
-        }
-        if constexpr (EPI == EPI_MULAUX) {
-            const int o = e_aux + 16 * i * p.ldaux + 32 * jp;
-            ld_x[0] = __builtin_amdgcn_raw_buffer_load_b32(raux, o, 0, 0);
-            ld_y[0] = __builtin_amdgcn_raw_buffer_load_b32(raux, o + 16, 0, 0);
-        }
-    };
-    auto epi_math = [&](auto cc, const f32x4 (&src)[4][4]) {
-        constexpr int c = decltype(cc)::value, jp = c >> 2, i = c & 3;
-        f32x4 vx = src[2 * jp][i], vy = src[2 * jp + 1][i];
-        if constexpr (DIAG == 1) {
-            asm volatile("" ::"v"(vx), "v"(vy));
-            return;
-        }
-        if constexpr (EPI == EPI_F32) {
-            const int o = e_c + (16 * i * p.ldc + 32 * jp) * 4;
-            vx = vx + (bias_x + __builtin_bit_cast(f32x4, ld_x));
-            vy = vy + (bias_y + __builtin_bit_cast(f32x4, ld_y));
-            __builtin_amdgcn_raw_buffer_store_b128(__builtin_bit_cast(u32x4, vx), rc_dst, o, 0, 0);
-            __builtin_amdgcn_raw_buffer_store_b128(__builtin_bit_cast(u32x4, vy), rc_dst, o + 64, 0, 0);
-            return;
-        } else {
-            if constexpr (EPI == EPI_GELU) {
-                vx += bias_x; vy += bias_y;
-                f32x4 cx, dx, cy, dy;
-                if constexpr (DIAG == 3) { cx = vx; dx = vx; cy = vy; dy = vy; }
-                else { gelu_cdf_pdf4(vx, cx, dx); gelu_cdf_pdf4(vy, cy, dy); }
-                const f32x4 gx = vx * dx + cx, gy = vy * dy + cy;
-                uint32_t bx = 0, by = 0;
-#pragma unroll
-                for (int e = 0; e < 4; ++e) {
-                    bx = __builtin_amdgcn_cvt_pk_u8_f32(__builtin_fmaf(gx[e], 200.f, 26.f), e, bx);
-                    by = __builtin_amdgcn_cvt_pk_u8_f32(__builtin_fmaf(gy[e], 200.f, 26.f), e, by);
-                }
-                swap16(bx, by);
-                if constexpr (DIAG == 2) asm volatile("" ::"v"(bx), "v"(by));
-                else __builtin_amdgcn_raw_buffer_store_b64((u32x2){bx, by}, raux, e_aux + 16 * i * p.ldaux + 32 * jp, 0, 0);
-                vx *= cx; vy *= cy;
-            }
-            if constexpr (EPI == EPI_MULAUX) {
-                vx *= unpack_dgelu_u8x4(ld_x[0]);
-                vy *= unpack_dgelu_u8x4(ld_y[0]);
-                if constexpr (i == 0) { cs_x = vx; cs_y = vy; } else { cs_x += vx; cs_y += vy; }
-                if constexpr (i == 3) {
-#pragma unroll
-                    for (int o = 1; o < 16; o <<= 1) {
-#pragma unroll
-                        for (int e = 0; e < 4; ++e) {
-                            cs_x[e] += __shfl_xor(cs_x[e], o, 64);
-                            cs_y[e] += __shfl_xor(cs_y[e], o, 64);
-                        }
-                    }
-                    __builtin_amdgcn_raw_buffer_store_b128(__builtin_bit_cast(u32x4, cs_x), rcs, e_cs + 128 * jp, 0, 0);
-                    __builtin_amdgcn_raw_buffer_store_b128(__builtin_bit_cast(u32x4, cs_y), rcs, e_cs + 128 * jp + 64, 0, 0);
-                }
-            }
-            uint32_t x0 = pack_bf2(vx[0], vx[1]), x1 = pack_bf2(vx[2], vx[3]);
-            uint32_t y0 = pack_bf2(vy[0], vy[1]), y1 = pack_bf2(vy[2], vy[3]);
-            swap16(x0, y0);
-            swap16(x1, y1);
-            if constexpr (DIAG == 2) asm volatile("" ::"v"(x0), "v"(x1), "v"(y0), "v"(y1));
-            else __builtin_amdgcn_raw_buffer_store_b128((u32x4){x0, x1, y0, y1}, rc_dst, e_c + (16 * i * p.ldc + 32 * jp) * 2, 0, 0);
-        }
-    };
+    EpiAcc<EPI, 4, DIAG> epi(p);
+    auto epi_setup = [&](int m0, int n0) { epi.template setup<2>(m0, n0, w_s); };
+    auto epi_loads = [&](auto cc) { epi.loads(cc); };
+    auto epi_math = [&](auto cc, const f32x4 (&src)[4][4]) { epi.math(cc, src); };
 
     auto kstep = [&](auto first_c, auto chunk_c) {
         constexpr bool FIRST = decltype(first_c)::value;
@@ -278,12 +170,12 @@
         auto fetch = [&](auto cc) {
             constexpr int c = decltype(cc)::value;
             epi_loads(cc);
-            tx[c] = ld_x; ty[c] = ld_y;
-            if constexpr ((c & 3) == 0) { tbx[c >> 2] = bias_x; tby[c >> 2] = bias_y; }
+            tx[c] = epi.ld_x; ty[c] = epi.ld_y;
+            if constexpr ((c & 3) == 0) { tbx[c >> 2] = epi.bias_x; tby[c >> 2] = epi.bias_y; }
         };
         auto finish = [&](auto cc) {
             constexpr int c = decltype(cc)::value;
-            ld_x = tx[c]; ld_y = ty[c]; bias_x = tbx[c >> 2]; bias_y = tby[c >> 2];
+            epi.ld_x = tx[c]; epi.ld_y = ty[c]; epi.bias_x = tbx[c >> 2]; epi.bias_y = tby[c >> 2];
             epi_math(cc, acc);
         };
         fetch(integral_constant<int, 0>{}); fetch(integral_constant<int, 1>{}); fetch(integral_constant<int, 2>{});
@@ -325,13 +217,7 @@
 
 }
 
-static int pp_epilogue(int flags) {
-    if (flags == 0) return EPI_BF16;
-    if (flags == (MH_GEMM_BIAS | MH_GEMM_GELU | MH_GEMM_AUX_DGELU | MH_GEMM_AUX_U8)) return EPI_GELU;
-    if (flags == (MH_GEMM_MULAUX | MH_GEMM_AUX_U8 | MH_GEMM_COLSUM)) return EPI_MULAUX;
-    if (flags == (MH_GEMM_OUT_F32 | MH_GEMM_BIAS | MH_GEMM_RESIDUAL)) return EPI_F32;
-    return -1;
-}
+static int pp_epilogue(int flags) { return epi_acc_form(flags); }
 
 bool gemm_pp_serves(int tile, int layout, const GemmParams& p) {
     const int epi = pp_epilogue(p.flags), diag = tile - MH_TILE_PP_128;
diff --git a/maestro_amd/engine.py b/maestro_amd/engine.py
--- a/maestro_amd/engine.py
+++ b/maestro_amd/engine.py
@@ -480,7 +480,7 @@
         self.group_streams = os.environ.get("MAESTRO_GROUP_STREAMS") != "0"
         self.tune_gemm = os.environ.get("MAESTRO_TUNE", "0") == "1"
         self.instep_tune = (os.environ.get("MAESTRO_INSTEP_TUNE", "0") == "1" and not self.tune_gemm
-                            and not any(os.environ.get(k) for k in ("MH_GEMM_TILE", "MH_GEMM_DMA", "MH_GEMM_PP", "MH_DMA_STAGGER")))
+                            and not any(os.environ.get(k) for k in ("MH_GEMM_TILE", "MH_GEMM_DMA", "MH_GEMM_PP", "MH_DMA_STAGGER", "MH_DMA_EPI")))
         self.tile_report = None
         self.warm_passes = 0
         self.warm_passes_run = 0
diff --git a/maestro_amd/hip.py b/maestro_amd/hip.py
--- a/maestro_amd/hip.py
+++ b/maestro_amd/hip.py
@@ -73,6 +73,7 @@
 
 TILE_AUTO, TILE_REG_128, TILE_DMA_256, TILE_DMA_256x128, TILE_DMA_128x256, TILE_DMA_128, TILE_DMA_128x4 = -1, 0, 1, 2, 3, 4, 5
 TILE_DMA_256_LOCKSTEP = 6
+TILE_DMA_256_EPI0, TILE_DMA_256_LOCKSTEP_EPI0 = 18, 19
 TILE_REG_64, TILE_REG_192 = 13, 14
 TILE_SK_192, TILE_SK_256, TILE_SK_DMA_256 = 15, 16, 17
 SK_TILES = (TILE_SK_192, TILE_SK_256, TILE_SK_DMA_256)
@@ -82,7 +83,8 @@
 _TILE_NAME = {TILE_REG_128: "gemm_kernel<{}>", TILE_DMA_256: "gemm_dma_kernel<256x256,{}>",
               TILE_DMA_256x128: "gemm_dma_kernel<256x128,{}>", TILE_DMA_128x256: "gemm_dma_kernel<128x256,{}>",
               TILE_DMA_128: "gemm_dma_kernel<128x128,{}>", TILE_DMA_128x4: "gemm_dma_kernel<128x128q,{}>",
-              TILE_DMA_256_LOCKSTEP: "gemm_dma_kernel<256x256,{}>", TILE_PP_128: "gemm_pp_kernel<{}>",
+              TILE_DMA_256_LOCKSTEP: "gemm_dma_kernel<256x256,{}>", TILE_DMA_256_EPI0: "gemm_dma_kernel<256x256,{}>",
+              TILE_DMA_256_LOCKSTEP_EPI0: "gemm_dma_kernel<256x256,{}>", TILE_PP_128: "gemm_pp_kernel<{}>",
               TILE_REG_64: "gemm_kernel<{},64x128>", TILE_REG_192: "gemm_kernel<{},192x128>",
               TILE_SK_192: "gemm_sk_kernel<{},192x128>", TILE_SK_256: "gemm_sk_kernel<{},256x128>",
               TILE_SK_DMA_256: "gemm_sk_dma_kernel<256x256,{}>"}
@@ -270,6 +272,17 @@
     return tile
 
 
+_EPI0 = {TILE_DMA_256: TILE_DMA_256_EPI0, TILE_DMA_256_LOCKSTEP: TILE_DMA_256_LOCKSTEP_EPI0}
+
+
+def _epi_switch(tile: int, args) -> int:
+    if _shape_only or os.environ.get("MH_DMA_EPI", "")[:1] != "0":
+        return tile
+    if tile == TILE_AUTO and _resolve(TILE_AUTO, args) == TILE_DMA_256:
+        tile = TILE_DMA_256
+    return _EPI0.get(tile, tile)
+
+
 def gemm(layout: int, M: int, N: int, K: int, A, lda: int, B, ldb: int, C, ldc: int, flags: int = 0, bias=None,
          res=None, ldr: int = 0, aux_in=None, aux_out=None, ldaux: int = 0, colsum=None, tile: int | None = None) -> None:
     args = (layout, M, N, K, A, lda, B, ldb, C, ldc, flags, bias, res, ldr, aux_in, aux_out, ldaux, colsum)
@@ -287,6 +300,7 @@
         return
     if not explicit:
         tile = _pick_tile(layout, M, N, K, flags, args)
+    tile = _epi_switch(tile, args)
     ev = None
     if _timer is not None:
         named = tile if tile in SK_TILES else _resolve(tile, args)
```

After: 1873 (median of 6 runs). About the same (+0.5%).
